# bacon205/Multimodal_eeg_fmri

Hardware: AMD Instinct MI355X
Metric: pairs_per_sec_per_node (higher is better)
Workload: dtype bf16

## Files before the change

### include/mmeeg_hip.h

```cpp
#ifndef MMEEG_HIP_H
#define MMEEG_HIP_H

#include <stdint.h>

#ifdef __cplusplus
extern "C" {
#endif

typedef struct ihipStream_t* hipStream_t;

#define MM_ABI_VERSION 5

const char* mm_last_error(void);
int mm_abi_version(void);

int mm_pack_nct_bf16(const float* x, void* y, int B, int C, int T, int Cp, hipStream_t stream);
int mm_unpack_ntc_f32(const void* g, float* dx, int B, int C, int T, int Cp, hipStream_t stream);
int mm_prep_conv_weight(const float* w, void* w_fwd, void* w_dgrad, int Cout, int Cin, int k,
                        int Cinp, int Coutp, hipStream_t stream);

int mm_conv1d_fwd(const void* x, const void* w, int B, int T, int Cin, int Cout, int taps, int pad,
                  const float* scale, const float* shift, int act, const float* residual,
                  const float* pe, int pool, float* stats, float* out_f32, void* out_bf16,
                  void* out_pre, float drop_p, uint32_t drop_seed, const uint32_t* seed_epoch,
                  const void* gradz, int gradz_act, hipStream_t stream);
int mm_conv1d_fwd_splitk_plan(int B, int T, int Cin, int Cout, int taps, int* nsplit_host, int64_t* ws_floats_host,
                              hipStream_t stream);
int mm_conv1d_fwd_splitk(const void* x, const void* w, int B, int T, int Cin, int Cout, int taps, int pad,
                  const float* scale, const float* shift, int act, const float* residual,
                  const float* pe, int pool, float* stats, float* out_f32, void* out_bf16,
                  void* out_pre, float drop_p, uint32_t drop_seed, const uint32_t* seed_epoch,
                  const void* gradz, int gradz_act, float* ws, int nsplit, hipStream_t stream);
int mm_conv1d_wgrad(const void* dy, const void* x, float* dw, float* dbias, int B, int T, int Cin,
                    int Cout, int taps, int pad, int Cin_real, int64_t sn, int64_t sc, int64_t stap,
                    int nrep, int64_t rep_stride, int slot_mode, hipStream_t stream);
int mm_conv1d_wgrad_slots(int B, int T, int Cin, int Cout, int taps, int* slots_host, hipStream_t stream);
int mm_conv1d_wgrad_many(const void* desc_host, int n, hipStream_t stream);
int mm_conv1d_wgrad_many_slots(int B, int T, int Cin, int Cout, int* slots_host, hipStream_t stream);
int mm_wgrad_scatter(const float* ws, float* dw, int Cout, int Cin, int taps, int Cinp, int nrep,
                     hipStream_t stream);
int mm_add_pe(const float* x, const float* pe, float* out_f32, void* out_bf16, int B, int L, int D,
              float drop_p, uint32_t seed, const uint32_t* seed_epoch, hipStream_t stream);

int mm_debug_stamp(void* buf, int idx, hipStream_t stream);
int mm_prep_many(const void* desc_host, int ndesc, hipStream_t stream);
int mm_prep_many_zero(const void* desc_host, int ndesc, float* zero, int64_t nzero, hipStream_t stream);
int mm_scatter_many(const void* desc_host, int ndesc, hipStream_t stream);
int mm_reduce_many(const void* desc_host, int ndesc, hipStream_t stream);
int mm_flush_many(const void* scatter_desc_host, int nscatter, const void* reduce_desc_host, int nreduce,
                  hipStream_t stream);
int mm_acc_reduce(const float* acc, float* dst, int K, int64_t rep_stride, hipStream_t stream);
int mm_reduce_replicas(const float* src, float* dst, int K, int nrep, int64_t rep_stride, hipStream_t stream);

int mm_bn_finalize(const float* stats, const float* gamma, const float* beta, float* run_mean,
                   float* run_var, const float* conv_bias, float* out4, int N, float count,
                   float momentum, float eps, int mode, void* batches_tracked, hipStream_t stream);
typedef struct {
    const float* stats;
    const float* gamma; const float* beta;
    float* run_mean; float* run_var;
    float* out4;
    void* batches_tracked;
    float count, momentum, eps;
    int reserved;
} mm_bn_fin_t;
int mm_bn_act_fwd_fin(const float* y, const void* bn_fin_host, const float* pe, void* out_bf16, float* out_f32,
                      int R, int S, int N, int act, int pool, int drop_first, float drop_p, uint32_t seed,
                      float drop2_p, uint32_t seed2, const uint32_t* seed_epoch, hipStream_t stream);
int mm_bn_act_fwd_ln_fin(const float* y, const void* bn_fin_host, const float* pe, float* out_f32, int R, int S,
                         int act, float drop_p, uint32_t seed, float drop2_p, uint32_t seed2,
                         const uint32_t* seed_epoch, const float* ln_gamma, const float* ln_beta, float ln_eps,
                         void* ln_out_bf16, float* ln_stat, hipStream_t stream);
int mm_pool3d_bn_act_fwd_fin(const void* y, const void* bn_fin_host, void* out_bf16, void* ysel, void* arg, int B,
                             int D, int H, int W, int N, int act, float drop_p, uint32_t seed,
                             const uint32_t* seed_epoch, hipStream_t stream);
int mm_conv3d_l1_fwd_fin(const float* x, const void* wimg, const float* bias, const void* bn_fin_host, void* out,
                         int B, int D, int H, int W, float drop_p, uint32_t seed, const uint32_t* seed_epoch,
                         hipStream_t stream);
int mm_bn_act_fwd(const float* y, const float* scale, const float* shift, const float* pe,
                  void* out_bf16, float* out_f32, int R, int S, int N, int act, int pool,
                  int drop_first, float drop_p, uint32_t seed, float drop2_p, uint32_t seed2,
                  const uint32_t* seed_epoch, hipStream_t stream);
int mm_bn_act_fwd_ln(const float* y, const float* scale, const float* shift, const float* pe, float* out_f32,
                     int R, int S, int act, float drop_p, uint32_t seed, float drop2_p, uint32_t seed2,
                     const uint32_t* seed_epoch, const float* ln_gamma, const float* ln_beta, float ln_eps,
                     void* ln_out_bf16, float* ln_stat, hipStream_t stream);
int mm_bn_act_bwd_reduce(const float* y, const float* out4, const void* dout_bf16,
                         const float* dout_f32, float* sums_out, int R, int S, int N, int act,
                         int pool, int drop_first, float drop_p, uint32_t seed, float drop2_p,
                         uint32_t seed2, const uint32_t* seed_epoch, hipStream_t stream);
int mm_bn_act_bwd_apply(const float* y, const float* out4, const void* dout_bf16,
                        const float* dout_f32, const float* sums, void* dy, float* dy_f32, int R,
                        int S, int N, int act, int pool, int drop_first, float drop_p, uint32_t seed,
                        float drop2_p, uint32_t seed2, const uint32_t* seed_epoch, int train, int sums_nrep, hipStream_t stream);

int mm_layernorm_fwd(const float* x, const float* gamma, const float* beta, void* out_bf16,
                     float* out_f32, float* stat, int M, int D, float eps, hipStream_t stream);
int mm_layernorm_bwd(const void* dy_bf16, const float* dy_f32, const float* x, const float* stat,
                     const float* gamma, const float* dres, float* dx, void* dx_bf16, float* dgb_repl,
                     int M, int D, float drop_p, uint32_t seed, const uint32_t* seed_epoch,
                     hipStream_t stream);
int mm_linear_dgrad_ln_bwd(const void* dy, const void* w, int M, int K, const float* x, const float* stat,
                           const float* gamma, const float* dres, float* dx, void* dx_bf16, float* dgb_repl,
                           float drop_p, uint32_t seed, const uint32_t* seed_epoch, hipStream_t stream);

int mm_conv1d_dgrad_bn_reduce(const void* dy, const void* w_dgrad, int B, int T, int Cin, int Cout, int taps, int pad,
                              void* dx_bf16, const float* y_below, const float* out4_below, float* sums_below, int act,
                              int pool, int drop_first, float drop_p, uint32_t seed, const uint32_t* seed_epoch,
                              hipStream_t stream);

int mm_linear_fwd_ln_gemm2(const void* x, const void* w, int M, int K, const float* bias, const float* residual,
                           float* out_f32, float drop_p, uint32_t seed, const uint32_t* seed_epoch,
                           const float* ln_gamma, const float* ln_beta, float ln_eps, void* ln_out_bf16, float* ln_stat,
                           const void* w2, const float* bias2, int n2, void* out2_bf16, hipStream_t stream);
int mm_linear_fwd_ln_gemm2_act(const void* x, const void* w, int M, int K, const float* bias, const float* residual,
                               float* out_f32, float drop_p, uint32_t seed, const uint32_t* seed_epoch,
                               const float* ln_gamma, const float* ln_beta, float ln_eps, void* ln_out_bf16,
                               float* ln_stat, const void* w2, const float* bias2, int n2, void* out2_bf16,
                               void* pre2_bf16, int act2, float drop2_p, uint32_t seed2, hipStream_t stream);
int mm_linear_dgrad_ln_bwd_gemm2(const void* dy, const void* w, int M, int K, const float* x, const float* stat,
                                 const float* gamma, const float* dres, float* dx, void* dx_bf16, float* dgb_repl,
                                 float drop_p, uint32_t seed, const uint32_t* seed_epoch, const void* w2, void* do_bf16,
                                 int dres_rows_per_sample, hipStream_t stream);
int mm_linear_dgrad_ln_bwd_bn_reduce(const void* dy, const void* w, int M, int K, const float* x, const float* stat,
                                     const float* gamma, const float* dres, float* dx, float* dgb_repl,
                                     const uint32_t* seed_epoch, const float* y_below, const float* out4_below,
                                     float* sums_below, int act, float bn_drop_p, uint32_t bn_seed, float bn_drop2_p,
                                     uint32_t bn_seed2, hipStream_t stream);

int mm_bn_act_bwd_reduce_bcast(const float* y, const float* out4, const float* dout_rows, float scale, float* sums_out,
                               int R, int S, int N, int act, float drop_p, uint32_t seed, const uint32_t* seed_epoch,
                               hipStream_t stream);
int mm_bn_act_bwd_apply_bcast(const float* y, const float* out4, const float* dout_rows, float scale, const float* sums,
                              void* dy, int R, int S, int N, int act, float drop_p, uint32_t seed,
                              const uint32_t* seed_epoch, int train, int sums_nrep, hipStream_t stream);

int mm_pooled_head_bwd_rows(const float* dout, const void* z_pre_bf16, const float* W, void* dz_bf16, float* rows_out,
                            void* dx_bf16, int B, int L, int D, int N, int act, float drop_p, uint32_t seed,
                            float emit_drop_p, uint32_t emit_seed, const uint32_t* seed_epoch, hipStream_t stream);

int mm_attn_fwd(const void* qkv, void* out, float* lse, int B, int L, int H, int head_dim,
                float scale, float drop_p, uint32_t seed, const uint32_t* seed_epoch,
                const float* attn_mask, int attn_mask_per_head, hipStream_t stream);
int mm_attn_bwd(const void* qkv, const void* out, const void* dout, const float* lse, void* dqkv,
                float* delta_ws, int B, int L, int H, int head_dim, float scale, float drop_p,
                uint32_t seed, const uint32_t* seed_epoch, const float* attn_mask, int attn_mask_per_head,
                hipStream_t stream);
int mm_attn_fwd_hd(const void* qkv, void* out, float* lse, int B, int L, int H, int head_dim,
                   float scale, float drop_p, uint32_t seed, const uint32_t* seed_epoch,
                   const float* attn_mask, int attn_mask_per_head, hipStream_t stream);
int mm_attn_bwd_hd(const void* qkv, const void* out, const void* dout, const float* lse, void* dqkv,
                   float* delta_ws, int B, int L, int H, int head_dim, float scale, float drop_p,
                   uint32_t seed, const uint32_t* seed_epoch, const float* attn_mask, int attn_mask_per_head,
                   hipStream_t stream);

int mm_colsum(const void* a_bf16, const float* a_f32, float* out, int M, int N, hipStream_t stream);
int mm_meanpool_fwd(const float* x, float* out_f32, void* out_bf16, int B, int L, int D, hipStream_t stream);
int mm_meanpool_bwd(const float* g, float* dx, int B, int L, int D, hipStream_t stream);
int mm_stage_inputs(const float* eeg, void* eeg_packed_bf16, float* eeg_copy, int B, int C, int T, int Cp,
                    float* fmri_dst, const float* fmri_src, int64_t fmri_n, hipStream_t stream);
int mm_eeg_augment_plan(const float* x, uint32_t* plan, int64_t plan_words, int B, int C, int T, float p_noise, float p_drop,
                        int n_drop, uint32_t s_noise, uint32_t s_drop, uint32_t s_keys, hipStream_t stream);
int mm_stage_inputs_aug(const float* eeg, uint32_t* plan, int64_t plan_words, void* eeg_packed_bf16, float* eeg_out_f32,
                        int B, int C, int T, int Cp, float noise_factor, uint32_t s_gauss_a, uint32_t s_gauss_b,
                        float* fmri_dst, const float* fmri_src, int64_t fmri_n, hipStream_t stream);
int mm_act_bwd(const float* g_f32, const void* g_bf16, const void* z, void* out, int64_t n, int act,
               float drop_p, uint32_t seed, const uint32_t* seed_epoch, hipStream_t stream);

int mm_pack_volume_bf16(const float* x, void* y, int64_t nvox, int Cp, hipStream_t stream);
int mm_conv3d_fwd(const void* x, const void* w, int B, int D, int H, int W, int Cin, int Cout,
                  const float* shift, float* stats, float* out_f32, void* out_bf16, hipStream_t stream);
int mm_conv3d_wgrad(const void* dy, const void* x, float* dw, float* dbias, int B, int D, int H, int W,
                    int Cin, int Cout, int Cin_real, int64_t sn, int64_t sc, int64_t stap, int nrep,
                    int64_t rep_stride, int slot_mode, hipStream_t stream);
int mm_conv3d_wgrad_slots(int B, int D, int H, int W, int Cin, int Cout, int* slots_host, hipStream_t stream);
int mm_pool3d_bn_act_fwd(const void* y, const float* out4, void* out_bf16, void* ysel, void* arg, int B, int D,
                         int H, int W, int N, int act, float drop_p, uint32_t seed, const uint32_t* seed_epoch,
                         hipStream_t stream);
int mm_pool3d_bn_act_bwd_reduce(const void* ysel, const float* out4, const void* dout_bf16, float* sums_out,
                                int B, int D, int H, int W, int N, int act, float drop_p, uint32_t seed,
                                const uint32_t* seed_epoch, hipStream_t stream);
int mm_pool3d_bn_act_bwd_apply(const void* y, const void* arg, const float* out4, const void* dout_bf16,
                               const float* sums, void* dy, int B, int D, int H, int W, int N, int act,
                               float drop_p, uint32_t seed, const uint32_t* seed_epoch, int train, int sums_nrep,
                               hipStream_t stream);

int mm_conv3d_l1(int mode, const float* x, const void* wimg, const float* bias, const float* out4,
                 const void* dout, const float* sums, float* stats, void* out, float* dw_tapmajor,
                 float* dbias, int B, int D, int H, int W, int train, float drop_p, uint32_t seed,
                 const uint32_t* seed_epoch, hipStream_t stream);
int mm_conv3d_l1_fwd_winners(const float* x, const void* wimg, const float* bias, const float* out4, void* out,
                             void* arg, int B, int D, int H, int W, int train, float drop_p, uint32_t seed,
                             const uint32_t* seed_epoch, hipStream_t stream);
int mm_conv3d_l1_gram(const float* x, const void* wimg, const float* bias, float* gram, float* stats, int B, int D,
                      int H, int W, hipStream_t stream);
int mm_conv3d_l1_bwd(const float* x, const void* wimg, const float* bias, const float* out4, const void* dout,
                     float* sums_out, float* a1, const float* gram, float* dw, float* dbias, int B, int D,
                     int H, int W, int train, float drop_p, uint32_t seed, const uint32_t* seed_epoch,
                     hipStream_t stream);

int mm_small_linear_fwd(const float* x, const float* W, const float* bias, const float* scale,
                        const float* shift, float* y, float* pre, int B, int K, int N, int act,
                        float drop_p, uint32_t seed, const uint32_t* seed_epoch, hipStream_t stream);
int mm_small_linear_bwd(const float* dy, const float* x, const float* W, float* dx, float* dW, float* db,
                        int B, int K, int N, hipStream_t stream);
int mm_act_f32(const float* z, float* y, int64_t n, int act, float drop_p, uint32_t seed, const uint32_t* seed_epoch, hipStream_t stream);
int mm_act_bwd_f32(const float* g, const float* z, float* out, int64_t n, int act, float drop_p,
                   uint32_t seed, const uint32_t* seed_epoch, hipStream_t stream);
int mm_colstats(const float* x, float* stats, int B, int N, hipStream_t stream);
int mm_proj_heads_fwd(const float* x_e, const float* W_e, const float* b_e, const float* g_e, const float* be_e,
                      int K_e, const float* x_f, const float* W_f, const float* b_f, const float* g_f,
                      const float* be_f, int K_f, float* z1, float* hn, float* stat, float* z, float* nrm, int B,
                      int N, float eps, float drop_p, uint32_t seed_e, uint32_t seed_f,
                      const uint32_t* seed_epoch, hipStream_t stream);
int mm_proj_heads_bwd(const float* dz, const float* z, const float* nrm, const float* hn, const float* z1,
                      const float* stat, const float* x_e, const float* W_e, const float* g_e, int K_e,
                      const float* x_f, const float* W_f, const float* g_f, int K_f, float* dx_e, float* dW_e,
                      float* db_e, float* dg_e, float* dbe_e, float* dx_f, float* dW_f, float* db_f, float* dg_f,
                      float* dbe_f, int B, int N, float drop_p, uint32_t seed_e, uint32_t seed_f,
                      const uint32_t* seed_epoch, hipStream_t stream);
int mm_clip_loss_own_rows(const float* z_all, const float* logit_scale, float* scal4, float* dz_local, float* ws,
                          int B, int Bg, int N, int row0, hipStream_t stream);
int mm_clip_loss_ws_floats(int B, int Bg, int* floats_host, hipStream_t stream);
int mm_clip_loss_own_rows_grouped(const float* z_all, const int* gid_all, const float* logit_scale, float* scal4,
                                  float* dz_local, float* ws, int B, int Bg, int N, int row0, hipStream_t stream);
int mm_clip_loss_grouped_ws_floats(int B, int Bg, int* floats_host, hipStream_t stream);

#define MM_RETRIEVAL_KMAX 16
#define MM_RETRIEVAL_NMAX (1 << 20)
int mm_retrieval(const float* Q, const float* G, const int* pos, int* ranks, int* topk_idx, float* topk_score,
                 float* ws, int Nq, int Ng, int D, int k, hipStream_t stream);
int mm_retrieval_ws_floats(int Nq, int Ng, int D, int k, int* floats_host, hipStream_t stream);
int mm_retrieval_grouped(const float* Q, const float* G, const int* qgid, const int* ggid, int* ranks, float* ws,
                         int Nq, int Ng, int D, hipStream_t stream);
int mm_retrieval_grouped_ws_floats(int Nq, int Ng, int D, int* floats_host, hipStream_t stream);

typedef struct {
    float* w[3]; float* b[3]; float* gamma[3]; float* beta[3]; float* run_mean[3]; float* run_var[3];
    void* batches_tracked[3];
    float* W; float* B; float* Gamma; float* Beta; float* Run_mean; float* Run_var;
    int cin; int k[3]; int cinp; int reserved;
} mm_power_merge_t;
int mm_power_merge(const void* desc_host, int mode, hipStream_t stream);

int mm_softmax2_concat(const float* a, const float* c, const float* pa, const float* pc, float* out, int B,
                       int Ha, int Hc, hipStream_t stream);
int mm_learned_fusion(const float* f0, const float* f1, const float* f2, const float* dyn,
                      const float* logits, const float* temperature, float* fused, float* weights, int B,
                      int H, int M, hipStream_t stream);
int mm_attn_1xk(const float* p0, const float* p1, const float* p2, const float* p3, int K, const float* dctx,
                float* ctx, float* attw, float* dp0, float* dp1, float* dp2, float* dp3, int B, int E,
                int nhead, float drop_p, uint32_t seed, const uint32_t* seed_epoch, int backward,
                hipStream_t stream);
int mm_add_f32(const float* a, const float* b, float* out, int64_t n, hipStream_t stream);
int mm_attn_1x2(const float* proj_e, const float* proj_f, float* ctx, float* attw, int B, int E, int nhead,
                hipStream_t stream);
int mm_attn_1x2_train(const float* proj_e, const float* proj_f, const float* dctx, float* ctx, float* attw,
                      float* dproj_e, float* dproj_f, int B, int E, int nhead, float drop_p, uint32_t seed,
                      const uint32_t* seed_epoch, int backward, hipStream_t stream);
int mm_learned_fusion_bwd(const float* f0, const float* f1, const float* f2, const float* dyn,
                          const float* logits, const float* temperature, const float* dfused, float* df0,
                          float* df1, float* df2, float* ddyn, float* dlogits, float* dtemp, int B, int H,
                          int M, hipStream_t stream);
int mm_softmax2_concat_bwd(const float* dout, const float* a, const float* c, const float* pa,
                           const float* pc, float* da, float* dc, float* dpa, float* dpc, int B, int Ha,
                           int Hc, hipStream_t stream);
int mm_weighted_ce(const float* logits, const void* target_i64, const float* class_weight, float* loss_out,
                   float* dlogits, int B, int C, hipStream_t stream);
int mm_focal_loss(const float* logits, const void* target_i64, float* loss_out, float* per_sample,
                  float* dlogits, int B, int C, float alpha, float gamma, float scale, hipStream_t stream);
int mm_gate2_mix(const float* g, const float* erp, const float* pw, const float* conn, float* comb,
                 float* gate, int B, int H, float boost, hipStream_t stream);
int mm_gate2_mix_bwd(const float* dcomb, const float* g, const float* erp, const float* pw, float* derp,
                     float* dpw, float* dconn, float* dg, int B, int H, float boost, hipStream_t stream);
int mm_smoothed_ce(const float* logits, const void* target_i64, float* loss_out, float* dlogits, int B,
                   int C, float smoothing, hipStream_t stream);
int mm_stft_power(const float* x, void* out_bf16, float* out_f32, int B, int C, int T, int nfft, int hop,
                  int ch_off, int ch_total, hipStream_t stream);
#define MM_ZSCORE_WS_DOUBLES 64
int mm_sample_zscore_bf16(const float* x, void* out_bf16, double* ws, int B, int rows, int ch_valid, int ch_total,
                          float eps, hipStream_t stream);
int mm_sample_zscore_bwd(const float* x, const void* g_bf16, float* dx, int B, int rows, int ch_valid, int ch_total,
                         float eps, hipStream_t stream);
int mm_stft_power_bwd(const float* x, const float* g_power, float* dx, int B, int C, int T, int nfft, int hop,
                      int ch_off, int ch_total, hipStream_t stream);
int mm_mul_f32(const float* a, const float* b, float* out, int64_t n, hipStream_t stream);
int mm_linear_fwd_meanpool(const void* x, const void* w, int M, int K, const float* bias, const float* residual,
                           float* out_f32, float drop_p, uint32_t seed, const uint32_t* seed_epoch, float* pool_out,
                           int rows_per_group, hipStream_t stream);
int mm_linear_fwd_ln(const void* x, const void* w, int M, int K, const float* bias, const float* residual,
                     float* out_f32, float drop_p, uint32_t seed, const uint32_t* seed_epoch, const float* ln_gamma,
                     const float* ln_beta, float ln_eps, void* ln_out_bf16, float* ln_stat, hipStream_t stream);
int mm_pooled_head_fwd(const float* pooled, const float* pooled_acc, const float* W, const float* bias, float* out, void* z_pre_bf16,
                       void* pooled_bf16, int B, int D, int N, int act, float drop_p, uint32_t seed,
                       const uint32_t* seed_epoch, hipStream_t stream);
int mm_pooled_head_bwd(const float* dout, const void* z_pre_bf16, const float* W, void* dz_bf16, float* dx,
                       void* dx_bf16, int B, int L, int D, int N, int act, float drop_p, uint32_t seed,
                       float emit_drop_p, uint32_t emit_seed, const uint32_t* seed_epoch, hipStream_t stream);
int mm_drop_path(const float* x, float* out, int64_t B, int64_t inner, float drop_p, uint32_t seed,
                 const uint32_t* seed_epoch, hipStream_t stream);
int mm_meanpool_bf16(const void* x, float* out, int R, int S, int N, hipStream_t stream);

#define MM_OPT_STATE_FLOATS 1032
int mm_sumsq(const float* g, float* state, int64_t n, hipStream_t stream);
int mm_adamw_clip(float* p, float* g, float* m, float* v, float* state, int64_t n, float beta1,
                  float beta2, float eps, float weight_decay, float max_norm, float grad_scale,
                  int zero_grad, uint32_t* seed_epoch, hipStream_t stream);

int mm_xai_interp(const float* x, const float* base, int base_rows, float* out, int n_steps, int s0, int steps,
                  int64_t rows, int64_t inner, hipStream_t stream);
int mm_xai_accum(const float* grad, float* acc, int steps, int64_t n, hipStream_t stream);
int mm_xai_finish(const float* x, const float* base, int base_rows, const float* acc, float* attr, float* chan,
                  int B, int C, int64_t T, int n_steps, int mode, hipStream_t stream);
int mm_xai_pair_score(const float* z, float* score, float* seed, int B, int N, hipStream_t stream);

int mm_gatv2_fwd(const float* xl, const float* xr, int ld, const float* att, const float* bias, const int* rowptr,
                 const int* col, float* out, float* pre, float* alpha, int B, int N, int H, int C, int E,
                 float slope, int act, float drop_p, uint32_t seed, const uint32_t* seed_epoch, hipStream_t stream);
int mm_gatv2_bwd(const float* dout, const float* pre, const float* xl, const float* xr, int ld, const float* att,
                 const float* alpha, const int* rowptr, const int* col, const int* colptr, const int* row,
                 const int* perm, float* dxl, float* dxr, float* datt, float* dbias, float* ds_ws, float* dz_ws,
                 float* part_ws, int B, int N, int H, int C, int E, float slope, int act, float drop_p,
                 uint32_t seed, const uint32_t* seed_epoch, hipStream_t stream);

int mm_gatv2_edge_fwd(const float* xl, const float* xr, int ld, const float* att, const float* bias,
                      const float* w_edge, const float* edge_attr, int ea_batched, const int* rowptr, const int* col,
                      float* out, float* pre, float* alpha, int B, int N, int H, int C, int E, int D, float slope,
                      int act, float drop_p, uint32_t seed, const uint32_t* seed_epoch, hipStream_t stream);
int mm_gatv2_edge_bwd(const float* dout, const float* pre, const float* xl, const float* xr, int ld, const float* att,
                      const float* w_edge, const float* edge_attr, int ea_batched, const float* alpha,
                      const int* rowptr, const int* col, const int* colptr, const int* row, const int* perm,
                      float* dxl, float* dxr, float* datt, float* dbias, float* dw_edge, float* dedge_attr,
                      float* ds_ws, float* dz_ws, float* part_ws, float* wpart_ws, float* epart_ws, int B, int N,
                      int H, int C, int E, int D, float slope, int act, float drop_p, uint32_t seed,
                      const uint32_t* seed_epoch, hipStream_t stream);
int mm_gatv2_edge_pack(const float* listed, const int* eid, const int* rowptr, const int* indeg, float* csr, int Bo,
                       int N, int El, int E, int D, int fill_mean, float fill_value, hipStream_t stream);
int mm_gatv2_edge_pack_bwd(const float* dcsr, const int* pos, const int* tgt, const int* rowptr, const int* indeg,
                           float* dlisted, int Bo, int N, int El, int E, int D, int fill_mean, hipStream_t stream);

#ifdef __cplusplus
}
#endif
#endif
```

### multimodal_eeg_fmri_amd/autograd.py

```python
from __future__ import annotations

import os
from typing import Dict, List, Optional

import torch

from . import _hip
from . import ops
from .ops import ACT, AREPL, REPL, WREP, _BF, _F32, _empty, _zeros


_BAG = {"cur": None}


def _reduce_into(dst, src, K, stride, offset=0, nrep=REPL):
    if dst is None:
        return
    if nrep not in (1, REPL):
        raise ValueError("_reduce_into: nrep is 1 (fp32 vector) or REPL (accumulator workspace)")
    bag = _BAG["cur"]
    ptr = src.data_ptr() + (8 if nrep == REPL else 4) * offset
    if bag is not None:
        bag.defer(ptr, dst, K, AREPL if nrep == REPL else 1, stride, keep=src)
    elif nrep == REPL:
# ... 20 lines not shown
    if window is None:
        return (ws.data_ptr(), dw.data_ptr(), cout, cin, taps, cinp, nrep, 0)
    n0, tap0, ws_taps, ws_cout = window
    return (ws.data_ptr() + 4 * n0 * ws_taps * cinp, dw.data_ptr(), cout, cin, taps | (tap0 << 8) | (ws_taps << 16), cinp, nrep, ws_cout)


def _wgrad_slots(dy, x, dw, dbr, B, T, cinp, N, k, pad, cin, parts=None):
    bag = _BAG["cur"]
    grouped = bag is not None and k == 1
    if grouped:
        slots = _hip.host_int("mm_conv1d_wgrad_many_slots", B, T, cinp, N)
    else:
        slots = _hip.host_int("mm_conv1d_wgrad_slots", B, T, cinp, N, k)
    ws = _empty((slots, N, k, cinp), _F32, dy)
    if grouped:
        bag.defer_wgrad(dy, x, ws, dbr, B, T, cinp, N, slots)
    elif bag is not None and bag.defer_conv_wgrads:
        bag.calls.append(("mm_conv1d_wgrad", (dy, x, ws, dbr, B, T, cinp, N, k, pad, cinp, k * cinp, 1, cinp,
                                              slots, N * k * cinp, 1)))
    else:
        _hip.call("mm_conv1d_wgrad", dy, x, ws, dbr, B, T, cinp, N, k, pad, cinp, k * cinp, 1, cinp,
                  slots, N * k * cinp, 1)
    if parts is None:
        _scatter_into(dw, ws, N, cin, k, cinp, slots)
    else:
        for t, n0, cn, kk in parts:
            if t is not None:
                _scatter_into(t, ws, cn, cin, kk, cinp, slots, window=(n0, (k - kk) // 2, k, N))


class deferred:

    def __init__(self, bag, device):
        self.bag, self.device = bag, device

    def __enter__(self):
        self.prev = _BAG["cur"]
        _BAG["cur"] = self.bag
        return self.bag

    def __exit__(self, *exc):
        _BAG["cur"] = self.prev
        if exc[0] is None:
            self.bag.flush(self.device)
        return False


def _ln_param_grads(bag, ln, dgb, D):
    gw, gb = bag.target(ln.weight), bag.target(ln.bias)
    if gw is not None and gb is not None and gw.data_ptr() + 4 * D == gb.data_ptr():
        _reduce_into(gw, dgb, 2 * D, 2 * D)
        return
    _reduce_into(gw, dgb, D, 2 * D, 0)
    _reduce_into(gb, dgb, D, 2 * D, D)


def _compact(rep_buf, K):
    out = _zeros((K,), rep_buf)
    _hip.call("mm_acc_reduce", rep_buf, out, K, K)
    return out


def _bn_param_grads(bag, bn, sums, N, nrep=1):
    _reduce_into(bag.target(bn.bias), sums, N, 2 * N, 0, nrep=nrep)
    _reduce_into(bag.target(bn.weight), sums, N, 2 * N, N, nrep=nrep)


class GradBag:

    def __init__(self):
        self.fresh: Dict[int, torch.Tensor] = {}
        self.pending = []
        self.scatters = []
        self.wgrads = []
        self.calls = []
        self.defer_conv_wgrads = False
        self._keep = []

    def defer(self, src_ptr: int, dst: torch.Tensor, K: int, nrep: int, stride: int, keep=None):
        self.pending.append((src_ptr, dst.data_ptr(), K, nrep, stride))
        self._keep.append((dst, keep))

    def defer_scatter(self, ws: torch.Tensor, dw: torch.Tensor, cout, cin, taps, cinp, nrep, window=None):
        self.scatters.append(scatter_desc(ws, dw, cout, cin, taps, cinp, nrep, window))
        self._keep.append((dw, ws))

    def defer_wgrad(self, dy, x, ws, dbr, B, T, cinp, N, slots):
        self.wgrads.append((dy.data_ptr(), x.data_ptr(), ws.data_ptr(), dbr.data_ptr() if dbr is not None else 0,
                            B, T, cinp, N, cinp, slots))
        self._keep.append((dy, x, ws, dbr))

    def hand_over(self) -> "GradBag":
        other = GradBag()
        other.pending, other.scatters, other.wgrads, other._keep = self.pending, self.scatters, self.wgrads, self._keep
        other.calls = self.calls
        self.pending, self.scatters, self.wgrads, self.calls, self._keep = [], [], [], [], []
        return other

    def flush(self, device):
        import ctypes
        import struct
        for name, args in self.calls:
            _hip.call(name, *args)
        self._keep.append(self.calls)
        self.calls = []
        if self.wgrads:
            raw = b"".join(struct.pack("<QQQQiiiiiiii", *d, 0, 0) for d in self.wgrads)
            host = ctypes.create_string_buffer(raw, len(raw))
            _hip.call("mm_conv1d_wgrad_many", ctypes.addressof(host), len(self.wgrads))
            self.wgrads = []
        if not self.scatters and not self.pending:
            return
        sraw = b"".join(struct.pack("<QQiiiiii", *d) for d in self.scatters)
        rraw = b"".join(struct.pack("<QQqqq", *d) for d in self.pending)
        shost = ctypes.create_string_buffer(sraw, max(len(sraw), 1))
        rhost = ctypes.create_string_buffer(rraw, max(len(rraw), 1))
        _hip.call("mm_flush_many", ctypes.addressof(shost) if self.scatters else None, len(self.scatters),
                  ctypes.addressof(rhost) if self.pending else None, len(self.pending))
        self.scatters, self.pending = [], []

    def target(self, p: torch.Tensor) -> Optional[torch.Tensor]:
        if p is None or not p.requires_grad:
            return None
        sink = getattr(p, "_mm_grad", None)
        if sink is not None:
            return sink
        t = self.fresh.get(id(p))
        if t is None:
            t = torch.zeros_like(p, dtype=_F32, memory_format=torch.contiguous_format)
            self.fresh[id(p)] = t
        return t

    def result(self, p: torch.Tensor) -> Optional[torch.Tensor]:
        return self.fresh.get(id(p))


def _mask_cast(g_f32=None, g_bf16=None, z=None, act="none", drop_p=0.0, seed=0):
    src = g_f32 if g_f32 is not None else g_bf16
    out = _empty(src.shape, _BF, src)
    _hip.call("mm_act_bwd", g_f32, g_bf16, z, out, src.numel(), ACT[act], float(drop_p), int(seed), ops.EP())
    return out


def linear_bwd(bag: GradBag, dy: torch.Tensor, x: torch.Tensor, weight, bias, *, need_dx=True,
               dx_f32=False, below=None):
    """dy (M, N) bf16, x (M, Kp) bf16 -> dx (M, Kp); accumulates dW, db."""
    M, N = dy.shape
    Kp = x.shape[1]
    K = weight.shape[1]
    dw = bag.target(weight)
    db = bag.target(bias)
    dbr = _zeros((REPL, N), dy) if db is not None else None
    if dw is not None:
        _wgrad_slots(dy, x, dw, dbr, 1, M, Kp, N, 1, 0, K)
    elif db is not None:
        _hip.call("mm_colsum", dy, None, dbr, M, N)
    if db is not None:
        _reduce_into(db, dbr, N, N)
    if not need_dx:
        return None
    _, wd, cinp, coutp = ops.weights.get(weight, True)
    if coutp != N:
        raise _hip.HipLibraryError(f"linear_bwd: dY width {N} != padded out width {coutp}")
    kw = {}
    if below is not None:
        z, act, p, seed = below
        kw = dict(gradz=z, gradz_act=act, drop_p=p, seed=seed)
    r = ops.igemm(dy.view(1, M, N), wd, 1, 0, cinp, out_f32=dx_f32, out_bf16=not dx_f32, **kw)
    return (r["f32"] if dx_f32 else r["bf16"]).view(M, cinp)


_NO_BCAST = bool(os.environ.get("MM_NO_BCAST"))
_NO_GEMM2 = bool(os.environ.get("MM_NO_GEMM2"))
_NO_BNRED = bool(os.environ.get("MM_NO_BNRED"))


def _bn_bwd_args(s: dict, y):
    B, T, N = y.shape
    d2 = s.get("drop2", (0.0, 0))
    return (B, T, N, ACT[s["act"]], s["pool"], 1 if s["drop_first"] else 0, float(s["drop_p"]), int(s["seed"]),
            float(d2[0]), int(d2[1]), ops.EP())


def conv_bn_act_bwd(bag: GradBag, s: dict, dout_bf16=None, dout_f32=None, need_dx=True, sums=None, below=None):
    conv, bn = s["conv"], s["bn"]
    y, out4, xb = s["y"], s["out4"], s["xb"]
    B, T, N = y.shape
    args = _bn_bwd_args(s, y)
    if sums is None:
        sums = _zeros((REPL, 2, N), y)
        _hip.call("mm_bn_act_bwd_reduce", y, out4, dout_bf16, dout_f32, sums, *args)
    dy = _empty((B, T, N), _BF, y)
    _hip.call("mm_bn_act_bwd_apply", y, out4, dout_bf16, dout_f32, sums, dy, None, *args,
              1 if s.get("train", True) else 0, REPL)
    _bn_param_grads(bag, bn, sums, N, nrep=REPL)
    k, pad = conv.kernel_size[0], conv.padding[0]
    cin = conv.in_channels
    parts = getattr(conv, "parts", None)
    if parts is not None:
        parts = [(bag.target(w), n0, w.shape[0], w.shape[2]) for w, n0 in parts]
        dw = None
    else:
        dw = bag.target(conv.weight)
    if dw is not None or (parts is not None and any(t is not None for t, *_ in parts)):
        cinp_x = xb.shape[2]
        db = bag.target(conv.bias)
        dbr = _zeros((REPL, N), y) if db is not None else None
        _wgrad_slots(dy, xb, dw, dbr, B, T, cinp_x, N, k, pad, cin, parts=parts)
        if db is not None:
            _reduce_into(db, dbr, N, N)
    if not need_dx:
        return None if below is None else (None, None)
    _, wd, cinp, coutp = ops.weights.get(conv.weight, True)
    assert coutp == N
    if below is not None:
        yb = below["y"]
        d2 = below.get("drop2", (0.0, 0))
        if not _NO_BNRED and (k > 1 or cinp <= 64) and yb.shape[2] == cinp and yb.shape[1] == T * below["pool"] and float(d2[0]) == 0.0:
            dx = _empty((B, T, cinp), _BF, y)
            sums_b = _zeros((REPL, 2, cinp), y)
            _hip.call("mm_conv1d_dgrad_bn_reduce", dy, wd, B, T, N, cinp, k, k - 1 - pad, dx, yb, below["out4"], sums_b,
                      ACT[below["act"]], below["pool"], 1 if below["drop_first"] else 0, float(below["drop_p"]),
                      int(below["seed"]), ops.EP())
            return dx, sums_b
        return ops.igemm(dy, wd, k, k - 1 - pad, cinp)["bf16"], None
    return ops.igemm(dy, wd, k, k - 1 - pad, cinp)["bf16"]


def _linear_ln_bwd(bag, dy, h, lin, wb, x, stat, ln, dres, dx, dx_bf16, dgb, drop_p, seed, bn_below=None, gemm2=None,
                   res_rows=0):
    weight, bias = (lin.weight, lin.bias) if lin is not None else wb
    M, D = x.shape
    if D == 128 and M % 32 == 0:
        linear_bwd(bag, dy, h, weight, bias, need_dx=False)
        _, wd, cinp, coutp = ops.weights.get(weight, True)
        if coutp != dy.shape[1] or cinp != D:
            raise _hip.HipLibraryError(f"linear_ln_bwd: dY width {dy.shape[1]} / LN width {D} != weight image {coutp} x {cinp}")
        if bn_below is not None and dx_bf16 is None and dx is not None and not _NO_BNRED:
            sb = bn_below["s"]
            yb = sb["y"]
            d2 = sb.get("drop2", (0.0, 0))
            if yb.shape[2] == 128 and sb["pool"] == 1 and yb.shape[0] * yb.shape[1] == M:
                sums_b = _zeros((REPL, 2, 128), yb)
                _hip.call("mm_linear_dgrad_ln_bwd_bn_reduce", dy, wd, M, coutp, x, stat, ln.weight, dres, dx, dgb, ops.EP(),
                          yb, sb["out4"], sums_b, ACT[sb["act"]], float(sb["drop_p"]), int(sb["seed"]), float(d2[0]), int(d2[1]))
                bn_below["sums"] = sums_b
                return
        if gemm2 is not None and dx_bf16 is not None and not _NO_GEMM2:
            w2, holder = gemm2
            do = _empty((M, 128), _BF, dy)
            _hip.call("mm_linear_dgrad_ln_bwd_gemm2", dy, wd, M, coutp, x, stat, ln.weight, dres, dx, dx_bf16, dgb,
                      drop_p, seed, ops.EP(), w2, do, int(res_rows))
            holder.append(do)
            return
        _hip.call("mm_linear_dgrad_ln_bwd", dy, wd, M, coutp, x, stat, ln.weight, dres, dx, dx_bf16, dgb,
                  drop_p, seed, ops.EP())
        return
    dh = linear_bwd(bag, dy, h, weight, bias)
    _hip.call("mm_layernorm_bwd", dh, None, x, stat, ln.weight, dres, dx, dx_bf16, dgb, M, D, drop_p, seed, ops.EP())


def transformer_block_bwd(bag: GradBag, s: dict, dx2: torch.Tensor, dy2=None, emit_for=None, bn_below=None):
    blk = s["blk"]
    p = s["p"]
    s1, s2, s3 = s["seeds"]
    B, L = s["B"], s["L"]
    at = blk.self_attn
    res_rows = 0
    if isinstance(dx2, tuple):
        rows, per = dx2
        M, D = dy2.shape
        _, _, ci, co = ops.weights.get(at.out_proj.weight, True)
        if D == 128 and M % 32 == 0 and ci == 128 and co == 128 and not _NO_GEMM2:
            dx2, res_rows = rows, per
        else:
            dx2 = rows.view(-1, 1, D).expand(-1, per, D).reshape(M, D).contiguous()
    else:
        M, D = dx2.shape
    if dy2 is None:
        dy2 = _mask_cast(g_f32=dx2, drop_p=p, seed=s3)
    dz = linear_bwd(bag, dy2, s["g"], blk.linear2.weight, blk.linear2.bias, below=(s["z"], blk._act, p, s2))
    dx1 = _empty((M, D), _F32, dx2)
    dyo = _empty((M, D), _BF, dx2)
    dgb = _zeros((REPL, 2, D), dx2)
    holder = []
    g2 = None
    if D == 128 and M % 32 == 0:
        _, wd_o, cinp_o, coutp_o = ops.weights.get(at.out_proj.weight, True)
        if cinp_o == 128 and coutp_o == 128:
            g2 = (wd_o, holder)
    _linear_ln_bwd(bag, dz, s["h2"], blk.linear1, None, s["x1"], s["st2"], blk.norm2, dx2, dx1, dyo, dgb,
                   float(p), int(s1), gemm2=g2, res_rows=res_rows)
    _ln_param_grads(bag, blk.norm2, dgb, D)
    if holder:
        do = holder[0]
        linear_bwd(bag, dyo, s["o"].view(M, D), at.out_proj.weight, at.out_proj.bias, need_dx=False)
    else:
        do = linear_bwd(bag, dyo, s["o"].view(M, D), at.out_proj.weight, at.out_proj.bias)
    dqkv = _empty((B, L, 3 * D), _BF, dx2)
    delta = _empty((B, blk.nhead, L), _F32, dx2)
    dh = D // blk.nhead
    pa, sa = s.get("attn_drop", (0.0, 0))
    entry = ops.attn_entry(D, blk.nhead, "bwd")
    _hip.call(entry, s["qkv"], s["o"], do, s["lse"], dqkv, delta, B, L, blk.nhead, dh, float(dh) ** -0.5,
              float(pa), int(sa), ops.EP(), s.get("mask"), ops.attn_mask_per_head(s.get("mask"), B, blk.nhead, L))
    dx0 = _empty((M, D), _F32, dx2)
    emit = _empty((M, D), _BF, dx2) if emit_for is not None else None
    ep, es = emit_for if emit_for is not None else (0.0, 0)
    dgb = _zeros((REPL, 2, D), dx2)
    _linear_ln_bwd(bag, dqkv.view(M, 3 * D), s["h1"], None, (at.in_proj_weight, at.in_proj_bias), s["x"], s["st1"],
                   blk.norm1, dx1, dx0, emit, dgb, float(ep), int(es), bn_below=bn_below)
    _ln_param_grads(bag, blk.norm1, dgb, D)
    return dx0, emit


def pooled_head_bwd(bag: GradBag, s: dict, dout: torch.Tensor, emit_for=None, rows_only=False):
    lin = s["lin"]
    if s.get("fused") and rows_only and emit_for is None and not _NO_BCAST:
        B, L, D = s["B"], s["L"], s["D"]
        N = lin.weight.shape[0]
        dout = dout.contiguous()
        dz = _empty((B, N), _BF, dout)
        dp = _empty((B, 1, D), _F32, dout)
        _hip.call("mm_pooled_head_bwd", dout, s["z"], lin.weight, dz, dp, None, B, 1, D, N, ACT[s["act"]],
                  float(s["drop_p"]), int(s["seed"]), 0.0, 0, ops.EP())
        linear_bwd(bag, dz, s["pooled"], lin.weight, lin.bias, need_dx=False)
        return dp.view(B, D), 1.0 / L
    if s.get("fused") and rows_only and emit_for is not None and not _NO_BCAST:
        B, L, D = s["B"], s["L"], s["D"]
        N = lin.weight.shape[0]
        dout = dout.contiguous()
        dz = _empty((B, N), _BF, dout)
        rows = _empty((B, D), _F32, dout)
        emit = _empty((B, L, D), _BF, dout)
        _hip.call("mm_pooled_head_bwd_rows", dout, s["z"], lin.weight, dz, rows, emit, B, L, D, N, ACT[s["act"]],
                  float(s["drop_p"]), int(s["seed"]), float(emit_for[0]), int(emit_for[1]), ops.EP())
        linear_bwd(bag, dz, s["pooled"], lin.weight, lin.bias, need_dx=False)
        return (rows, L), emit
    if s.get("fused"):
        B, L, D = s["B"], s["L"], s["D"]
        N = lin.weight.shape[0]
        dout = dout.contiguous()
        dz = _empty((B, N), _BF, dout)
        dx = _empty((B, L, D), _F32, dout)
        emit = _empty((B, L, D), _BF, dout) if emit_for is not None else None
        ep, es = emit_for if emit_for is not None else (0.0, 0)
        _hip.call("mm_pooled_head_bwd", dout, s["z"], lin.weight, dz, dx, emit, B, L, D, N, ACT[s["act"]],
                  float(s["drop_p"]), int(s["seed"]), float(ep), int(es), ops.EP())
        linear_bwd(bag, dz, s["pooled"], lin.weight, lin.bias, need_dx=False)
        return (dx, emit) if emit_for is not None else dx
    if emit_for is not None:
        return pooled_head_bwd(bag, s, dout), None
    dz = _mask_cast(g_f32=dout.contiguous(), z=s["z"], act=s["act"], drop_p=s["drop_p"], seed=s["seed"])
    dpool = linear_bwd(bag, dz, s["pooled"], lin.weight, lin.bias, dx_f32=True)
    B, L, D = s["B"], s["L"], s["D"]
    dx = _empty((B, L, D), _F32, dout)
    _hip.call("mm_meanpool_bwd", dpool, dx, B, L, D)
    return dx


def _module_params(m) -> List[torch.nn.Parameter]:
    return [p for p in m.parameters()]


class _ModuleFn(torch.autograd.Function):

    @staticmethod
    def _finish(ctx, bag, params, dx):
        return (None, dx) + tuple(bag.result(p) for p in params)


def erp_encoder_bwd(bag: GradBag, sv: dict, dout: torch.Tensor, need_dx: bool = False, after_blocks=None,
                    after_conv2=None, after_conv3=None):
    blocks = sv["blocks"]
    dy2 = None
    if blocks:
        d, dy2 = pooled_head_bwd(bag, sv["head"], dout, emit_for=(blocks[-1]["p"], blocks[-1]["seeds"][2]), rows_only=True)
    else:
        d = pooled_head_bwd(bag, sv["head"], dout)
    if isinstance(d, tuple):
        B, L, D = dy2.shape
    else:
        B, L, D = d.shape
        d = d.view(B * L, D)
    if dy2 is not None:
        dy2 = dy2.view(B * L, D)
    c3, c2, c1 = sv["convs"][2], sv["convs"][1], sv["convs"][0]
    bn3 = {"s": c3}
    for i in range(len(blocks) - 1, -1, -1):
        below = (blocks[i - 1]["p"], blocks[i - 1]["seeds"][2]) if i > 0 else None
        d, dy2 = transformer_block_bwd(bag, blocks[i], d, dy2=dy2, emit_for=below, bn_below=bn3 if i == 0 else None)
    if after_blocks is not None:
        after_blocks()
    g, sm = conv_bn_act_bwd(bag, c3, dout_f32=d.view(B, L, D), sums=bn3.get("sums"), below=c2)
    if after_conv3 is not None:
        after_conv3()
    g, sm = conv_bn_act_bwd(bag, c2, dout_bf16=g, sums=sm, below=c1)
    if after_conv2 is not None:
        after_conv2()
    g = conv_bn_act_bwd(bag, c1, dout_bf16=g, need_dx=need_dx, sums=sm)
    if not need_dx:
        return None
    Bx, C, T = sv["x_shape"]
    dx = _empty((Bx, C, T), _F32, dout)
    _hip.call("mm_unpack_ntc_f32", g, dx, Bx, C, T, g.shape[2])
    return dx


class ErpEncoderFn(_ModuleFn):

    @staticmethod
    def run(m, x):
        return ErpEncoderFn.apply(m, x, *_module_params(m))

    @staticmethod
    def forward(ctx, m, x, *params):
        out, saved = ops._erp_forward_impl(m, x.float(), m.training, True, save=True)
        ctx.m, ctx.saved, ctx.params = m, saved, params
        ctx.need_dx = x.requires_grad
        return out

    @staticmethod
    def backward(ctx, dout):
        bag = GradBag()
        with deferred(bag, dout.device):
            dx = erp_encoder_bwd(bag, ctx.saved, dout, ctx.need_dx)
        return _ModuleFn._finish(ctx, bag, ctx.params, dx)


def power_encoder_bwd(bag: GradBag, sv: dict, dout: torch.Tensor, need_dx: bool = False):
    d = pooled_head_bwd(bag, sv["head"], dout)
    B, L, D = d.shape
    d = d.view(B * L, D)
    blocks = sv["blocks"]
    dy2 = None
    for i in range(len(blocks) - 1, -1, -1):
        below = (blocks[i - 1]["p"], blocks[i - 1]["seeds"][2]) if i > 0 else None
        d, dy2 = transformer_block_bwd(bag, blocks[i], d, dy2=dy2, emit_for=below)
    g = conv_bn_act_bwd(bag, sv["convs"][1], dout_f32=d.view(B, L, D))
    g = conv_bn_act_bwd(bag, sv["convs"][0], dout_bf16=g, need_dx=need_dx)
    conv, bn, seqs = sv["merged"]

    def finish():
        tg = lambda ps: [bag.target(p) for p in ps]
        none3 = [None] * 3
        ops.power_merge_call(2, (tg([sq[0].weight for sq in seqs]), tg([sq[0].bias for sq in seqs]), tg([sq[1].weight for sq in seqs]),
                                 tg([sq[1].bias for sq in seqs]), none3, none3),
                             [bag.result(conv.weight), bag.result(conv.bias), bag.result(bn.weight), bag.result(bn.bias), None, None],
                             cin=conv.in_channels, ks=[sq[0].kernel_size[0] for sq in seqs])
    return g, finish


class PowerEncoderFn(_ModuleFn):

    @staticmethod
    def run(m, x, packed=False):
        return PowerEncoderFn.apply(m, x, packed, *_module_params(m))

    @staticmethod
    def forward(ctx, m, x, packed, *params):
        xb = x if packed else ops.pack_nct(x.float())
        need_dx = bool(x.requires_grad)
        out, saved = ops._power_forward_impl(m, xb, m.training, need_dx, save=True)
        ctx.saved, ctx.params = saved, params
        ctx.need_dx, ctx.x_shape, ctx.packed = need_dx, tuple(x.shape), bool(packed)
        return out

    @staticmethod
    def backward(ctx, dout):
        bag = GradBag()
        with deferred(bag, dout.device):
            g, finish = power_encoder_bwd(bag, ctx.saved, dout.contiguous(), ctx.need_dx)
        finish()
        dx = None
        if ctx.need_dx and ctx.packed:
            dx = g
        elif ctx.need_dx:
            Bx, C, T = ctx.x_shape
            dx = _empty((Bx, C, T), _F32, dout)
            _hip.call("mm_unpack_ntc_f32", g, dx, Bx, C, T, g.shape[2])
        return (None, dx, None) + tuple(bag.result(p) for p in ctx.params)


class StftFrontEndFn(torch.autograd.Function):

    @staticmethod
    def forward(ctx, x, n_ffts, hop, normalize):
        xc = x.float().contiguous()
        out, spec = ops.stft_front_end(xc, n_ffts, hop, normalize, keep_spec=True)
        ctx.save_for_backward(xc, spec if spec is not None else out)
        ctx.cfg = (tuple(n_ffts), int(hop), bool(normalize))
        return out

    @staticmethod
    def backward(ctx, g):
        xc, spec = ctx.saved_tensors
        n_ffts, hop, normalize = ctx.cfg
        B, C, T = xc.shape
        frames, cp = g.shape[1], g.shape[2]
        widths = [C * (n // 2 + 1) for n in n_ffts]
        g = g.contiguous()
        if normalize:
            gp = _empty((B, frames, cp), _F32, g)
            _hip.call("mm_sample_zscore_bwd", spec, g, gp, B, frames, sum(widths), cp, 1e-8)
        else:
            gp = g.float()
        dx = torch.zeros_like(xc)
        off = 0
        for n, wdt in zip(n_ffts, widths):
            _hip.call("mm_stft_power_bwd", xc, gp, dx, B, C, T, int(n), hop, off, cp)
            off += wdt
        return dx, None, None, None


class AddPositionalFn(torch.autograd.Function):

    @staticmethod
    def forward(ctx, x, pe, p):
        seed = ops._next_seed() if p > 0 else 0
        ctx.p, ctx.seed, ctx.dtype = p, seed, x.dtype
        return ops.add_positional_impl(x, pe, p, seed)

    @staticmethod
    def backward(ctx, dout):
        if ctx.p > 0:
            dx = ops.add_positional_impl(dout, None, ctx.p, ctx.seed, backward=True)
        else:
            dx = dout
        return dx.to(ctx.dtype), None, None


class TransformerBlockFn(_ModuleFn):
    @staticmethod
    def run(blk, x, mask=None):
        return TransformerBlockFn.apply(blk, x, mask, *_module_params(blk))

    @staticmethod
    def forward(ctx, blk, x, mask, *params):
        xf = x.float().contiguous()
        out, saved = ops.transformer_block_fwd(xf, blk, blk.training, True, save=True, mask=mask)
        ctx.blk, ctx.saved, ctx.params = blk, saved, params
        return out

    @staticmethod
    def backward(ctx, dout):
        bag = GradBag()
        B, L, D = dout.shape
        with deferred(bag, dout.device):
            dx, _ = transformer_block_bwd(bag, ctx.saved, dout.contiguous().view(B * L, D).float())
        return (None, dx.view(B, L, D), None) + tuple(bag.result(p) for p in ctx.params)


def conv3d_bn_act_bwd(bag: GradBag, s: dict, dout, need_dx=True):
    conv, bn = s["conv"], s["bn"]
    y, out4, xv = s["y"], s["out4"], s["xv"]
    B, D, H, W, N = y.shape
    train = 1 if s.get("train", True) else 0
    sums = _zeros((REPL, 2, N), y)
    dy = _empty((B, D, H, W, N), _BF, y)
    gelu = ACT["gelu"]
    if s["pool"]:
        _hip.call("mm_pool3d_bn_act_bwd_reduce", s["ysel"], out4, dout, sums, B, D, H, W, N, gelu,
                  float(s["drop_p"]), int(s["seed"]), ops.EP())
        _hip.call("mm_pool3d_bn_act_bwd_apply", y, s["arg"], out4, dout, sums, dy, B, D, H, W, N, gelu,
                  float(s["drop_p"]), int(s["seed"]), ops.EP(), train, REPL)
    elif isinstance(dout, tuple):
        rows, scale = dout
        _hip.call("mm_bn_act_bwd_reduce_bcast", y, out4, rows, float(scale), sums, B, D * H * W, N, gelu,
                  float(s["drop_p"]), int(s["seed"]), ops.EP())
        _hip.call("mm_bn_act_bwd_apply_bcast", y, out4, rows, float(scale), sums, dy, B, D * H * W, N, gelu,
                  float(s["drop_p"]), int(s["seed"]), ops.EP(), train, REPL)
    else:
        args = (B, D * H * W, N, gelu, 1, 1, float(s["drop_p"]), int(s["seed"]), 0.0, 0, ops.EP())
        _hip.call("mm_bn_act_bwd_reduce", y, out4, None, dout, sums, *args)
        _hip.call("mm_bn_act_bwd_apply", y, out4, None, dout, sums, dy, None, *args, train, REPL)
    _bn_param_grads(bag, bn, sums, N, nrep=REPL)
    cin = conv.in_channels
    dw = bag.target(conv.weight)
    if dw is not None:
        cinp_x = xv.shape[4]
        db = bag.target(conv.bias)
        dbr = _zeros((REPL, N), y) if db is not None else None
        slots = _hip.host_int("mm_conv3d_wgrad_slots", B, D, H, W, cinp_x, N)
        ws = _empty((slots, N, 27, cinp_x), _F32, y)
        end = ops.kernel_timer.bracket(f"conv3d_wgrad_c{cinp_x}")
        _hip.call("mm_conv3d_wgrad", dy, xv, ws, dbr, B, D, H, W, cinp_x, N, cinp_x,
                  27 * cinp_x, 1, cinp_x, slots, N * 27 * cinp_x, 1)
        if end is not None:
            end.record()
        _scatter_into(dw, ws, N, cin, 27, cinp_x, slots)
        if db is not None:
            _reduce_into(db, dbr, N, N)
    if not need_dx:
        return None
    _, wd, cinp, coutp = ops.weights.get(conv.weight, True)
    assert coutp == N
    dx = _empty((B, D, H, W, cinp), _BF, y)
    end = ops.kernel_timer.bracket(f"conv3d_dgrad_c{N}")
    _hip.call("mm_conv3d_fwd", dy, wd, B, D, H, W, N, cinp, None, None, None, dx)
    if end is not None:
        end.record()
    return dx


def conv3d_l1_bwd(bag: GradBag, s: dict, dout: torch.Tensor):
    conv, bn, x = s["conv"], s["bn"], s["x"]
    B, _, D, H, W = x.shape
    train = 1 if s.get("train", True) else 0
# ... 125 lines not shown
```

### multimodal_eeg_fmri_amd/csrc/attention.hip

```cpp
#include "common.h"

namespace {

constexpr int VR = 32;

__device__ __forceinline__ bf16x8 tr_frag32(const bf16* tile, int row0, int lane) {
    const int li = lane & 15, g = lane >> 4;
    const bf16* p = tile + (row0 + 8 * (g >> 1) + (li >> 2)) * VR + (g & 1) * 16 + 4 * (li & 3);
    typedef __attribute__((address_space(3))) s16x4 lds_s16x4;
    union { s16x4 s[2]; bf16x8 v; } u;
    u.s[0] = __builtin_amdgcn_ds_read_tr16_b64_v4i16((lds_s16x4*)(p));
    u.s[1] = __builtin_amdgcn_ds_read_tr16_b64_v4i16((lds_s16x4*)(p + 4 * VR));
    return u.v;
}

__device__ __forceinline__ int vperm(int key) {
    return (key & ~12) | ((key & 4) << 1) | ((key & 8) >> 1);
}

__device__ __forceinline__ uint32_t attn_block_hash(uint32_t seed, int bh, int q, int key, int L) {
    const uint32_t Lh = ((uint32_t)L + 1u) >> 1;
    uint32_t x = (((uint32_t)bh * Lh + ((uint32_t)q >> 1)) * Lh + ((uint32_t)key >> 1)) * 0x9E3779B1u + seed;
    x ^= x >> 13;
    x = __umul24(x, 0xB5297Bu);
    x ^= x >> 15;
    return x;
}
template <bool ALONG_KEYS>
__device__ __forceinline__ void attn_keep2(uint32_t seed, int bh, int mine, int other, int L, uint32_t thresh8, bool& k0, bool& k1) {
    if (ALONG_KEYS) {
        const uint32_t x = attn_block_hash(seed, bh, mine, other, L) >> (16 * (mine & 1));
        k0 = (x & 0xFFu) >= thresh8;
        k1 = ((x >> 8) & 0xFFu) >= thresh8;
    } else {
        const uint32_t x = attn_block_hash(seed, bh, other, mine, L) >> (8 * (mine & 1));
        k0 = (x & 0xFFu) >= thresh8;
        k1 = ((x >> 16) & 0xFFu) >= thresh8;
    }
}

__device__ __forceinline__ float xhalf_max(float v) {
    const auto r = __builtin_amdgcn_permlane32_swap(__float_as_uint(v), __float_as_uint(v), false, false);
    return fmaxf(__uint_as_float(r[0]), __uint_as_float(r[1]));
}
__device__ __forceinline__ float xhalf_sum(float v) {
    const auto r = __builtin_amdgcn_permlane32_swap(__float_as_uint(v), __float_as_uint(v), false, false);
    return __uint_as_float(r[0]) + __uint_as_float(r[1]);
}

__device__ __forceinline__ float fast_exp2(float x) { return __builtin_amdgcn_exp2f(x); }

__device__ __forceinline__ void zero8(bf16x8& v) {
#pragma unroll
    for (int j = 0; j < 8; ++j) v[j] = (bf16)0.f;
}

constexpr int KCH = 128;
constexpr int QCH = 128;

template <int DHP>
struct Hd {
    static_assert(DHP == 32 || DHP == 64, "padded head width");
    static constexpr int NS = DHP / 16;
    static constexpr int NT = DHP / 32;
    static constexpr int KS = DHP + 8;
    static constexpr int NG = DHP / 8;
    static __device__ __forceinline__ int tr_off(int rows, int row, int sg) { return (sg >> 2) * rows * VR + row * VR + (sg & 3) * 8; }
};

template <int DHP, bool EXACT>
struct Dims {
    int L, H, dh_;
    Dims(int L, int H, int dh) : L(L), H(H), dh_(dh) {}
    __device__ int dh() const { return dh_; }
};
template <int DHP>
struct Dims<DHP, true> {
    int L, H;
    Dims(int L, int H, int) : L(L), H(H) {}
    __device__ constexpr int dh() const { return DHP; }
};

template <int DHP, bool EXACT, bool DROP, bool FULL, bool MASK>
__global__ __launch_bounds__(256) void attn_fwd_kernel(const bf16* __restrict__ qkv, bf16* __restrict__ out,
                                                       float* __restrict__ lse, const Dims<DHP, EXACT> dm, float scale_log2,
                                                       uint32_t dthresh, uint32_t dseed, float dinv,
                                                       const uint32_t* epoch, const float* __restrict__ amask, size_t amask_bh) {
    using T = Hd<DHP>;
    constexpr int NS = T::NS, NT = T::NT, KS = T::KS, NG = T::NG;
    const int L = dm.L, H = dm.H, dh = dm.dh();
    dseed = mm_eff_seed(dseed, epoch);
    if (MASK) amask += (size_t)(blockIdx.z * H + blockIdx.y) * amask_bh;
    __shared__ __attribute__((aligned(16))) bf16 Ks[KCH * KS];
    __shared__ __attribute__((aligned(16))) bf16 Vs[NT * KCH * VR];
    const int E = H * dh, E3 = 3 * E;
    const int b = blockIdx.z, h = blockIdx.y;
    const int tid = threadIdx.x, lane = tid & 63, wave = tid >> 6;
    const int lr = lane & 31, lh = lane >> 5;
    const int q = blockIdx.x * 128 + wave * 32 + lr;
    const bf16* base = qkv + (size_t)b * L * E3 + h * dh;

    bf16x8 qf[NS];
#pragma unroll
    for (int s = 0; s < NS; ++s) {
        zero8(qf[s]);
        if (q < L && 16 * s + 8 * lh < dh) qf[s] = *reinterpret_cast<const bf16x8*>(base + (size_t)q * E3 + 16 * s + 8 * lh);
    }
    f32x16 o[NT];
#pragma unroll
    for (int t = 0; t < NT; ++t)
#pragma unroll
        for (int r = 0; r < 16; ++r) o[t][r] = 0.f;
    float m_run = -INFINITY, l_run = 0.f;

    constexpr int NI = KCH * NG / 256;
    uint4 kreg[NI], vreg[NI];
    auto load_chunk = [&](int k0) __attribute__((always_inline)) {
        const int kn = min(KCH, L - k0);
#pragma unroll
        for (int i = 0; i < NI; ++i) {
            const int s = tid + i * 256, key = s / NG, sg = s % NG;
            kreg[i] = make_uint4(0, 0, 0, 0); vreg[i] = make_uint4(0, 0, 0, 0);
            if (key < kn && sg * 8 < dh) {
                const bf16* row = base + (size_t)(k0 + key) * E3;
                kreg[i] = *reinterpret_cast<const uint4*>(row + E + sg * 8);
                vreg[i] = *reinterpret_cast<const uint4*>(row + 2 * E + sg * 8);
            }
        }
    };
    load_chunk(0);
#pragma unroll
    for (int s = 0; s < NS; ++s) asm volatile("" : : "v"(qf[s]));
    for (int k0 = 0; k0 < L; k0 += KCH) {
        const int kn = min(KCH, L - k0);
        const int kn32 = (kn + 31) & ~31;
        __syncthreads();
#pragma unroll
        for (int i = 0; i < NI; ++i) {
            const int s = tid + i * 256, key = s / NG, sg = s % NG;
            if (key >= kn32) continue;
            *reinterpret_cast<uint4*>(Ks + key * KS + sg * 8) = kreg[i];
            *reinterpret_cast<uint4*>(Vs + T::tr_off(KCH, vperm(key), sg)) = vreg[i];
        }
        __syncthreads();
        if (k0 + KCH < L) load_chunk(k0 + KCH);
        bf16x8 kfr[NS];
#pragma unroll
        for (int s = 0; s < NS; ++s) kfr[s] = *reinterpret_cast<const bf16x8*>(Ks + lr * KS + 16 * s + 8 * lh);
        for (int kt = 0; kt < kn32; kt += 32) {
            f32x16 sacc;
#pragma unroll
            for (int r = 0; r < 16; ++r) sacc[r] = 0.f;
#pragma unroll
            for (int s = 0; s < NS; ++s) sacc = __builtin_amdgcn_mfma_f32_32x32x16_bf16(kfr[s], qf[s], sacc, 0, 0, 0);
            bf16x8 vfr[NT][2];
#pragma unroll
            for (int t = 0; t < NT; ++t)
#pragma unroll
                for (int s = 0; s < 2; ++s) vfr[t][s] = tr_frag32(Vs + t * KCH * VR, kt + 16 * s, lane);
            if (kt + 32 < kn32)
#pragma unroll
                for (int s = 0; s < NS; ++s) kfr[s] = *reinterpret_cast<const bf16x8*>(Ks + (kt + 32 + lr) * KS + 16 * s + 8 * lh);
            const float sc2 = MASK ? 1.f : scale_log2;
            float mx = -INFINITY;
#pragma unroll
            for (int r = 0; r < 16; ++r) {
                const int key = kt + (r & 3) + 8 * (r >> 2) + 4 * lh;
                float sc = sacc[r];
                if (MASK) {
                    sc *= scale_log2;
                    if (key < kn) sc += amask[(size_t)min(q, L - 1) * L + k0 + key] * 1.4426950408889634f;
                }
                sacc[r] = (FULL || key < kn) ? sc : -INFINITY;
                mx = fmaxf(mx, sacc[r]);
            }
            mx = xhalf_max(mx);
            if (__builtin_amdgcn_ballot_w64(mx * sc2 > m_run + 8.f)) {
                const float m_new = fmaxf(m_run, mx * sc2);
                const float alpha = fast_exp2(m_run - ((MASK && m_new == -INFINITY) ? 0.f : m_new));
                l_run *= alpha;
                m_run = m_new;
#pragma unroll
                for (int t = 0; t < NT; ++t)
#pragma unroll
                    for (int r = 0; r < 16; ++r) o[t][r] *= alpha;
            }
            const float m_neg = (MASK && m_run == -INFINITY) ? 0.f : -m_run;
            float ps = 0.f;
            union { bf16x8 v[2]; bf16x2 h[8]; } pu;
#pragma unroll
            for (int r = 0; r < 16; r += 2) {
                float p0 = fast_exp2(fmaf(sacc[r], sc2, m_neg)), p1 = fast_exp2(fmaf(sacc[r + 1], sc2, m_neg));
                ps += p0;
                ps += p1;
                if (DROP) {
                    bool kp0, kp1;
                    attn_keep2<true>(dseed, b * H + h, q, k0 + kt + (r & 3) + 8 * (r >> 2) + 4 * lh, L, dthresh, kp0, kp1);
                    p0 = kp0 ? p0 : 0.f; p1 = kp1 ? p1 : 0.f;
                }
                typedef __attribute__((ext_vector_type(2))) float f32x2_t;
                pu.h[r >> 1] = __builtin_convertvector((f32x2_t){p0, p1}, bf16x2);
            }
            l_run += ps;
#pragma unroll
            for (int t = 0; t < NT; ++t)
#pragma unroll
                for (int s = 0; s < 2; ++s) o[t] = __builtin_amdgcn_mfma_f32_32x32x16_bf16(vfr[t][s], pu.v[s], o[t], 0, 0, 0);
        }
    }
    const float l_tot = xhalf_sum(l_run);
    const float inv = (DROP ? dinv : 1.f) / l_tot;
    if (q < L) {
        bf16* orow = out + ((size_t)b * L + q) * E + h * dh;
#pragma unroll
        for (int t = 0; t < NT; ++t)
#pragma unroll
            for (int g = 0; g < 4; ++g) {
                const int d = 32 * t + 8 * g + 4 * lh;
                if (d >= dh) continue;
                bf16x4 v = {(bf16)(o[t][4 * g] * inv), (bf16)(o[t][4 * g + 1] * inv), (bf16)(o[t][4 * g + 2] * inv), (bf16)(o[t][4 * g + 3] * inv)};
                *reinterpret_cast<bf16x4*>(orow + d) = v;
            }
        if (lse && lh == 0) lse[((size_t)b * H + h) * L + q] = (m_run + log2f(l_tot)) * 0.6931471805599453f;
    }
}

template <int DHP, bool EXACT, bool DROP, bool FULL, bool MASK>
__global__ __launch_bounds__(256) void attn_bwd_dq_kernel(const bf16* __restrict__ qkv, const bf16* __restrict__ out,
                                                          const bf16* __restrict__ dout, const float* __restrict__ lse,
                                                          bf16* __restrict__ dqkv, float* __restrict__ delta,
                                                          const Dims<DHP, EXACT> dm, float scale, uint32_t dthresh,
                                                          uint32_t dseed, float dinv, const uint32_t* epoch,
                                                          const float* __restrict__ amask, size_t amask_bh) {
    using T = Hd<DHP>;
    constexpr int NS = T::NS, NT = T::NT, KS = T::KS, NG = T::NG;
    const int L = dm.L, H = dm.H, dh = dm.dh();
    dseed = mm_eff_seed(dseed, epoch);
    if (MASK) amask += (size_t)(blockIdx.z * H + blockIdx.y) * amask_bh;
    __shared__ __attribute__((aligned(16))) bf16 Ks[KCH * KS];
    __shared__ __attribute__((aligned(16))) bf16 Vs[KCH * KS];
    __shared__ __attribute__((aligned(16))) bf16 Kr[NT * KCH * VR];
    const int E = H * dh, E3 = 3 * E;
    const int b = blockIdx.z, h = blockIdx.y;
    const int tid = threadIdx.x, lane = tid & 63, wave = tid >> 6;
    const int lr = lane & 31, lh = lane >> 5;
    const int q = blockIdx.x * 128 + wave * 32 + lr;
    const bool qok = q < L;
    const bf16* base = qkv + (size_t)b * L * E3 + h * dh;
    const float scale_log2 = scale * 1.4426950408889634f;

    bf16x8 qf[NS], dof[NS];
    float dl = 0.f;
#pragma unroll
    for (int s = 0; s < NS; ++s) {
        zero8(qf[s]); zero8(dof[s]);
        if (qok && 16 * s + 8 * lh < dh) {
            qf[s] = *reinterpret_cast<const bf16x8*>(base + (size_t)q * E3 + 16 * s + 8 * lh);
            const size_t oi = ((size_t)b * L + q) * E + h * dh + 16 * s + 8 * lh;
            dof[s] = *reinterpret_cast<const bf16x8*>(dout + oi);
            const bf16x8 of = *reinterpret_cast<const bf16x8*>(out + oi);
#pragma unroll
            for (int j = 0; j < 8; ++j) dl += (float)dof[s][j] * (float)of[j];
        }
    }
    dl = xhalf_sum(dl);
    const float lse2 = qok ? lse[((size_t)b * H + h) * L + q] * 1.4426950408889634f : 0.f;
    if (qok && lh == 0) delta[((size_t)b * H + h) * L + q] = dl;

    f32x16 dq[NT];
#pragma unroll
    for (int t = 0; t < NT; ++t)
#pragma unroll
        for (int r = 0; r < 16; ++r) dq[t][r] = 0.f;

    constexpr int NI = KCH * NG / 256;
    uint4 kreg[NI], vreg[NI];
    auto load_chunk = [&](int k0) __attribute__((always_inline)) {
        const int kn = min(KCH, L - k0);
#pragma unroll
        for (int i = 0; i < NI; ++i) {
            const int s = tid + i * 256, key = s / NG, sg = s % NG;
            kreg[i] = make_uint4(0, 0, 0, 0); vreg[i] = make_uint4(0, 0, 0, 0);
            if (key < kn && sg * 8 < dh) {
                const bf16* row = base + (size_t)(k0 + key) * E3;
                kreg[i] = *reinterpret_cast<const uint4*>(row + E + sg * 8);
                vreg[i] = *reinterpret_cast<const uint4*>(row + 2 * E + sg * 8);
            }
        }
    };
    load_chunk(0);
#pragma unroll
    for (int s = 0; s < NS; ++s) asm volatile("" : : "v"(qf[s]), "v"(dof[s]));
    asm volatile("" : : "v"(dl), "v"(lse2));
    for (int k0 = 0; k0 < L; k0 += KCH) {
        const int kn = min(KCH, L - k0);
        const int kn32 = (kn + 31) & ~31;
        __syncthreads();
#pragma unroll
        for (int i = 0; i < NI; ++i) {
            const int s = tid + i * 256, key = s / NG, sg = s % NG;
            if (key >= kn32) continue;
            *reinterpret_cast<uint4*>(Ks + key * KS + sg * 8) = kreg[i];
            *reinterpret_cast<uint4*>(Vs + key * KS + sg * 8) = vreg[i];
            *reinterpret_cast<uint4*>(Kr + T::tr_off(KCH, vperm(key), sg)) = kreg[i];
        }
        __syncthreads();
        if (k0 + KCH < L) load_chunk(k0 + KCH);
        for (int kt = 0; kt < kn32; kt += 32) {
            f32x16 sacc, dp;
#pragma unroll
            for (int r = 0; r < 16; ++r) { sacc[r] = 0.f; dp[r] = 0.f; }
            bf16x8 kfr[NS], vfr[NS];
#pragma unroll
            for (int s = 0; s < NS; ++s) {
                kfr[s] = *reinterpret_cast<const bf16x8*>(Ks + (kt + lr) * KS + 16 * s + 8 * lh);
                vfr[s] = *reinterpret_cast<const bf16x8*>(Vs + (kt + lr) * KS + 16 * s + 8 * lh);
            }
#pragma unroll
            for (int s = 0; s < NS; ++s) {
                sacc = __builtin_amdgcn_mfma_f32_32x32x16_bf16(kfr[s], qf[s], sacc, 0, 0, 0);
                dp = __builtin_amdgcn_mfma_f32_32x32x16_bf16(vfr[s], dof[s], dp, 0, 0, 0);
            }
            bf16x8 ktfr[NT][2];
#pragma unroll
            for (int t = 0; t < NT; ++t)
#pragma unroll
                for (int s = 0; s < 2; ++s) ktfr[t][s] = tr_frag32(Kr + t * KCH * VR, kt + 16 * s, lane);
            bf16x8 dsf[2];
            bool kp[16];
            if (DROP)
#pragma unroll
                for (int r = 0; r < 16; r += 2)
                    attn_keep2<true>(dseed, b * H + h, q, k0 + kt + (r & 3) + 8 * (r >> 2) + 4 * lh, L, dthresh, kp[r], kp[r + 1]);
#pragma unroll
            for (int r = 0; r < 16; ++r) {
                const int key = kt + (r & 3) + 8 * (r >> 2) + 4 * lh;
                float sc = fmaf(sacc[r], scale_log2, -lse2);
                if (MASK && key < kn) sc += amask[(size_t)min(q, L - 1) * L + k0 + key] * 1.4426950408889634f;
                const float p = (FULL || key < kn) ? fast_exp2(sc) : 0.f;
                float dpr = dp[r];
                if (DROP) dpr = fmaf(kp[r] ? dpr : 0.f, dinv, -dl);
                else dpr -= dl;
                dsf[r >> 3][r & 7] = (bf16)(p * dpr);
            }
#pragma unroll
            for (int t = 0; t < NT; ++t)
#pragma unroll
                for (int s = 0; s < 2; ++s) dq[t] = __builtin_amdgcn_mfma_f32_32x32x16_bf16(ktfr[t][s], dsf[s], dq[t], 0, 0, 0);
        }
    }
    if (qok) {
        bf16* drow = dqkv + ((size_t)b * L + q) * E3 + h * dh;
#pragma unroll
        for (int t = 0; t < NT; ++t)
#pragma unroll
            for (int g = 0; g < 4; ++g) {
                const int d = 32 * t + 8 * g + 4 * lh;
                if (d >= dh) continue;
                bf16x4 v = {(bf16)(dq[t][4 * g] * scale), (bf16)(dq[t][4 * g + 1] * scale), (bf16)(dq[t][4 * g + 2] * scale), (bf16)(dq[t][4 * g + 3] * scale)};
                *reinterpret_cast<bf16x4*>(drow + d) = v;
            }
    }
}

template <int DHP, bool EXACT, bool DROP, bool FULL, bool MASK>
__global__ __launch_bounds__(256) void attn_bwd_dkv_kernel(const bf16* __restrict__ qkv, const bf16* __restrict__ dout,
                                                           const float* __restrict__ lse, const float* __restrict__ delta,
                                                           bf16* __restrict__ dqkv, const Dims<DHP, EXACT> dm, float scale,
                                                           uint32_t dthresh, uint32_t dseed, float dinv,
                                                           const uint32_t* epoch, const float* __restrict__ amask, size_t amask_bh) {
    using T = Hd<DHP>;
    constexpr int NS = T::NS, NT = T::NT, KS = T::KS, NG = T::NG;
    const int L = dm.L, H = dm.H, dh = dm.dh();
    dseed = mm_eff_seed(dseed, epoch);
    if (MASK) amask += (size_t)(blockIdx.z * H + blockIdx.y) * amask_bh;
    __shared__ __attribute__((aligned(16))) bf16 Qs[QCH * KS];
    __shared__ __attribute__((aligned(16))) bf16 Ds[QCH * KS];
    __shared__ __attribute__((aligned(16))) bf16 Qr[NT * QCH * VR];
    __shared__ __attribute__((aligned(16))) bf16 Dr[NT * QCH * VR];
    __shared__ float Ls[QCH], Dl[QCH];
    const int E = H * dh, E3 = 3 * E;
    const int b = blockIdx.z, h = blockIdx.y;
    const int tid = threadIdx.x, lane = tid & 63, wave = tid >> 6;
    const int lr = lane & 31, lh = lane >> 5;
    const int key = blockIdx.x * 128 + wave * 32 + lr;
    const bool kok = key < L;
    const bf16* base = qkv + (size_t)b * L * E3 + h * dh;
    const float scale_log2 = scale * 1.4426950408889634f;

    bf16x8 kf[NS], vf[NS];
#pragma unroll
    for (int s = 0; s < NS; ++s) {
        zero8(kf[s]); zero8(vf[s]);
        if (kok && 16 * s + 8 * lh < dh) {
            kf[s] = *reinterpret_cast<const bf16x8*>(base + (size_t)key * E3 + E + 16 * s + 8 * lh);
            vf[s] = *reinterpret_cast<const bf16x8*>(base + (size_t)key * E3 + 2 * E + 16 * s + 8 * lh);
        }
    }
    f32x16 dk[NT], dv[NT];
#pragma unroll
    for (int t = 0; t < NT; ++t)
#pragma unroll
        for (int r = 0; r < 16; ++r) { dk[t][r] = 0.f; dv[t][r] = 0.f; }

    constexpr int NI = QCH * NG / 256;
    static_assert(QCH <= 256, "one lse / delta value per thread");
    uint4 qreg[NI], dreg[NI];
    float lreg = INFINITY, dlreg = 0.f;
    auto load_chunk = [&](int q0) __attribute__((always_inline)) {
        const int qn = min(QCH, L - q0);
#pragma unroll
        for (int i = 0; i < NI; ++i) {
            const int s = tid + i * 256, qi = s / NG, sg = s % NG;
            qreg[i] = make_uint4(0, 0, 0, 0); dreg[i] = make_uint4(0, 0, 0, 0);
            if (qi < qn && sg * 8 < dh) {
                qreg[i] = *reinterpret_cast<const uint4*>(base + (size_t)(q0 + qi) * E3 + sg * 8);
                dreg[i] = *reinterpret_cast<const uint4*>(dout + ((size_t)b * L + q0 + qi) * E + h * dh + sg * 8);
            }
        }
        const bool ok = tid < qn;
        lreg = ok ? lse[((size_t)b * H + h) * L + q0 + tid] : INFINITY;
        dlreg = ok ? delta[((size_t)b * H + h) * L + q0 + tid] : 0.f;
    };
    load_chunk(0);
#pragma unroll
    for (int s = 0; s < NS; ++s) asm volatile("" : : "v"(kf[s]), "v"(vf[s]));
    for (int q0 = 0; q0 < L; q0 += QCH) {
        const int qn = min(QCH, L - q0);
        const int qn32 = (qn + 31) & ~31;
        __syncthreads();
#pragma unroll
        for (int i = 0; i < NI; ++i) {
            const int s = tid + i * 256, qi = s / NG, sg = s % NG;
            if (qi >= qn32) continue;
            *reinterpret_cast<uint4*>(Qs + qi * KS + sg * 8) = qreg[i];
            *reinterpret_cast<uint4*>(Ds + qi * KS + sg * 8) = dreg[i];
            *reinterpret_cast<uint4*>(Qr + T::tr_off(QCH, vperm(qi), sg)) = qreg[i];
            *reinterpret_cast<uint4*>(Dr + T::tr_off(QCH, vperm(qi), sg)) = dreg[i];
        }
        if (tid < qn32) { Ls[tid] = lreg * 1.4426950408889634f; Dl[tid] = dlreg; }
        __syncthreads();
        if (q0 + QCH < L) load_chunk(q0 + QCH);
        for (int qt = 0; qt < qn32; qt += 32) {
            f32x16 sacc, dp;
#pragma unroll
            for (int r = 0; r < 16; ++r) { sacc[r] = 0.f; dp[r] = 0.f; }
            bf16x8 qar[NS], dar[NS];
#pragma unroll
            for (int s = 0; s < NS; ++s) {
                qar[s] = *reinterpret_cast<const bf16x8*>(Qs + (qt + lr) * KS + 16 * s + 8 * lh);
                dar[s] = *reinterpret_cast<const bf16x8*>(Ds + (qt + lr) * KS + 16 * s + 8 * lh);
            }
#pragma unroll
            for (int s = 0; s < NS; ++s) {
                sacc = __builtin_amdgcn_mfma_f32_32x32x16_bf16(qar[s], kf[s], sacc, 0, 0, 0);
                dp = __builtin_amdgcn_mfma_f32_32x32x16_bf16(dar[s], vf[s], dp, 0, 0, 0);
            }
            bf16x8 dtar[NT][2], qtar[NT][2];
#pragma unroll
            for (int t = 0; t < NT; ++t)
#pragma unroll
                for (int s = 0; s < 2; ++s) {
                    dtar[t][s] = tr_frag32(Dr + t * QCH * VR, qt + 16 * s, lane);
                    qtar[t][s] = tr_frag32(Qr + t * QCH * VR, qt + 16 * s, lane);
                }
            bf16x8 pf[2], dsf[2];
            bool kp[16];
            if (DROP)
#pragma unroll
                for (int r = 0; r < 16; r += 2)
                    attn_keep2<false>(dseed, b * H + h, key, q0 + qt + (r & 3) + 8 * (r >> 2) + 4 * lh, L, dthresh, kp[r], kp[r + 1]);
#pragma unroll
            for (int r = 0; r < 16; ++r) {
                const int qi = qt + (r & 3) + 8 * (r >> 2) + 4 * lh;
                float sc = fmaf(sacc[r], scale_log2, -Ls[qi]);
                if (MASK && kok && qi < qn) sc += amask[(size_t)(q0 + qi) * L + key] * 1.4426950408889634f;
                const float p = (FULL || kok) ? fast_exp2(sc) : 0.f;
                pf[r >> 3][r & 7] = (bf16)((!DROP || kp[r]) ? p : 0.f);
                const float u = DROP ? fmaf(kp[r] ? dp[r] : 0.f, dinv, -Dl[qi]) : dp[r] - Dl[qi];
                dsf[r >> 3][r & 7] = (bf16)(p * u);
            }
#pragma unroll
            for (int t = 0; t < NT; ++t)
#pragma unroll
                for (int s = 0; s < 2; ++s) {
                    dv[t] = __builtin_amdgcn_mfma_f32_32x32x16_bf16(dtar[t][s], pf[s], dv[t], 0, 0, 0);
                    dk[t] = __builtin_amdgcn_mfma_f32_32x32x16_bf16(qtar[t][s], dsf[s], dk[t], 0, 0, 0);
                }
        }
    }
    if (kok) {
        bf16* krow = dqkv + ((size_t)b * L + key) * E3 + E + h * dh;
        bf16* vrow = krow + E;
        const float dvs = DROP ? dinv : 1.f;
#pragma unroll
        for (int t = 0; t < NT; ++t)
#pragma unroll
            for (int g = 0; g < 4; ++g) {
                const int d = 32 * t + 8 * g + 4 * lh;
                if (d >= dh) continue;
                bf16x4 a = {(bf16)(dk[t][4 * g] * scale), (bf16)(dk[t][4 * g + 1] * scale), (bf16)(dk[t][4 * g + 2] * scale), (bf16)(dk[t][4 * g + 3] * scale)};
                bf16x4 c = {(bf16)(dv[t][4 * g] * dvs), (bf16)(dv[t][4 * g + 1] * dvs), (bf16)(dv[t][4 * g + 2] * dvs), (bf16)(dv[t][4 * g + 3] * dvs)};
                *reinterpret_cast<bf16x4*>(krow + d) = a;
                *reinterpret_cast<bf16x4*>(vrow + d) = c;
            }
    }
}

uint32_t attn_thresh(float p) { return p > 0.f ? (uint32_t)((double)p * 256.0 + 0.5) : 0u; }
float attn_keep_scale(uint32_t t) { return t ? 256.f / (256.f - (float)t) : 1.f; }

bool hd_supported(int dh) { return dh >= 16 && dh <= 64 && dh % 8 == 0; }

template <int DHP, bool EXACT>
void launch_fwd(const void* qkv, void* out, float* lse, int B, int L, int H, int dh, float scale, float drop_p,
                uint32_t seed, const uint32_t* seed_epoch, const float* attn_mask, int per_head, hipStream_t st) {
    const uint32_t dth = attn_thresh(drop_p);
    const size_t mask_bh = attn_mask && per_head ? (size_t)L * L : 0;
    const bool full = L % KCH == 0;
    auto kern = dth ? (full ? attn_fwd_kernel<DHP, EXACT, true, true, false> : attn_fwd_kernel<DHP, EXACT, true, false, false>)
                    : (full ? attn_fwd_kernel<DHP, EXACT, false, true, false> : attn_fwd_kernel<DHP, EXACT, false, false, false>);
    if (attn_mask) kern = dth ? attn_fwd_kernel<DHP, EXACT, true, false, true> : attn_fwd_kernel<DHP, EXACT, false, false, true>;
    hipLaunchKernelGGL(kern, dim3(ceil_div(L, 128), H, B), dim3(256), 0, st, (const bf16*)qkv, (bf16*)out, lse,
                       Dims<DHP, EXACT>(L, H, dh), scale * 1.4426950408889634f, dth, seed, attn_keep_scale(dth), seed_epoch,
                       attn_mask, mask_bh);
}

template <int DHP, bool EXACT>
int launch_bwd(const void* qkv, const void* out, const void* dout, const float* lse, void* dqkv, float* delta_ws,
               int B, int L, int H, int dh, float scale, float drop_p, uint32_t seed, const uint32_t* seed_epoch,
               const float* attn_mask, int per_head, hipStream_t st) {
    const uint32_t dth = attn_thresh(drop_p);
    const float dinv = attn_keep_scale(dth);
    const size_t mask_bh = attn_mask && per_head ? (size_t)L * L : 0;
    const bool full = L % KCH == 0 && L % QCH == 0;
    auto kdq = dth ? (full ? attn_bwd_dq_kernel<DHP, EXACT, true, true, false> : attn_bwd_dq_kernel<DHP, EXACT, true, false, false>)
                   : (full ? attn_bwd_dq_kernel<DHP, EXACT, false, true, false> : attn_bwd_dq_kernel<DHP, EXACT, false, false, false>);
    auto kdkv = dth ? (full ? attn_bwd_dkv_kernel<DHP, EXACT, true, true, false> : attn_bwd_dkv_kernel<DHP, EXACT, true, false, false>)
                    : (full ? attn_bwd_dkv_kernel<DHP, EXACT, false, true, false> : attn_bwd_dkv_kernel<DHP, EXACT, false, false, false>);
    if (attn_mask) {
        kdq = dth ? attn_bwd_dq_kernel<DHP, EXACT, true, false, true> : attn_bwd_dq_kernel<DHP, EXACT, false, false, true>;
        kdkv = dth ? attn_bwd_dkv_kernel<DHP, EXACT, true, false, true> : attn_bwd_dkv_kernel<DHP, EXACT, false, false, true>;
    }
    const dim3 grid(ceil_div(L, 128), H, B);
    const Dims<DHP, EXACT> dm(L, H, dh);
    hipLaunchKernelGGL(kdq, grid, dim3(256), 0, st, (const bf16*)qkv, (const bf16*)out, (const bf16*)dout, lse,
                       (bf16*)dqkv, delta_ws, dm, scale, dth, seed, dinv, seed_epoch, attn_mask, mask_bh);
    int rc = mm_check_launch(EXACT ? "attn_bwd_dq" : "attn_bwd_hd_dq");
    if (rc) return rc;
    hipLaunchKernelGGL(kdkv, grid, dim3(256), 0, st, (const bf16*)qkv, (const bf16*)dout, lse, delta_ws, (bf16*)dqkv,
                       dm, scale, dth, seed, dinv, seed_epoch, attn_mask, mask_bh);
    return mm_check_launch(EXACT ? "attn_bwd_dkv" : "attn_bwd_hd_dkv");
}

}

extern "C" {

int mm_attn_fwd(const void* qkv, void* out, float* lse, int B, int L, int H, int head_dim, float scale,
                float drop_p, uint32_t seed, const uint32_t* seed_epoch, const float* attn_mask, int attn_mask_per_head,
                hipStream_t st) {
    MM_REQUIRE(drop_p >= 0.f && drop_p < 1.f, "attn_fwd: drop_p");
    MM_REQUIRE(qkv && out && B > 0 && L > 0 && H > 0, "attn_fwd: null/invalid");
    MM_REQUIRE(head_dim == 32, "attn_fwd: head_dim=%d (kernel is specialised for 32)", head_dim);
    launch_fwd<32, true>(qkv, out, lse, B, L, H, head_dim, scale, drop_p, seed, seed_epoch, attn_mask, attn_mask_per_head, st);
    return mm_check_launch("attn_fwd");
}

int mm_attn_bwd(const void* qkv, const void* out, const void* dout, const float* lse, void* dqkv, float* delta_ws,
                int B, int L, int H, int head_dim, float scale, float drop_p, uint32_t seed,
                const uint32_t* seed_epoch, const float* attn_mask, int attn_mask_per_head, hipStream_t st) {
    MM_REQUIRE(qkv && out && dout && lse && dqkv && delta_ws && B > 0 && L > 0 && H > 0, "attn_bwd: null/invalid");
    MM_REQUIRE(head_dim == 32, "attn_bwd: head_dim=%d (kernel is specialised for 32)", head_dim);
    return launch_bwd<32, true>(qkv, out, dout, lse, dqkv, delta_ws, B, L, H, head_dim, scale, drop_p, seed, seed_epoch,
                                attn_mask, attn_mask_per_head, st);
}

int mm_attn_fwd_hd(const void* qkv, void* out, float* lse, int B, int L, int H, int head_dim, float scale,
                   float drop_p, uint32_t seed, const uint32_t* seed_epoch, const float* attn_mask, int attn_mask_per_head,
                   hipStream_t st) {
    MM_REQUIRE(hd_supported(head_dim), "attn_fwd_hd: head_dim=%d (supported: multiples of 8 in [16, 64])", head_dim);
    MM_REQUIRE(drop_p >= 0.f && drop_p < 1.f, "attn_fwd_hd: drop_p");
    MM_REQUIRE(qkv && out && B > 0 && L > 0 && H > 0, "attn_fwd_hd: null/invalid");
    auto launch = head_dim <= 32 ? launch_fwd<32, false> : launch_fwd<64, false>;
    launch(qkv, out, lse, B, L, H, head_dim, scale, drop_p, seed, seed_epoch, attn_mask, attn_mask_per_head, st);
    return mm_check_launch("attn_fwd_hd");
}

int mm_attn_bwd_hd(const void* qkv, const void* out, const void* dout, const float* lse, void* dqkv, float* delta_ws,
                   int B, int L, int H, int head_dim, float scale, float drop_p, uint32_t seed,
                   const uint32_t* seed_epoch, const float* attn_mask, int attn_mask_per_head, hipStream_t st) {
    MM_REQUIRE(hd_supported(head_dim), "attn_bwd_hd: head_dim=%d (supported: multiples of 8 in [16, 64])", head_dim);
    MM_REQUIRE(drop_p >= 0.f && drop_p < 1.f, "attn_bwd_hd: drop_p");
    MM_REQUIRE(qkv && out && dout && lse && dqkv && delta_ws && B > 0 && L > 0 && H > 0, "attn_bwd_hd: null/invalid");
    auto launch = head_dim <= 32 ? launch_bwd<32, false> : launch_bwd<64, false>;
    return launch(qkv, out, dout, lse, dqkv, delta_ws, B, L, H, head_dim, scale, drop_p, seed, seed_epoch, attn_mask,
                  attn_mask_per_head, st);
}

}
```

### multimodal_eeg_fmri_amd/csrc/common.h

```cpp
#pragma once
#include <hip/hip_runtime.h>
#include <stdint.h>

typedef __bf16 bf16;
typedef __attribute__((ext_vector_type(8))) __bf16 bf16x8;
typedef __attribute__((ext_vector_type(4))) __bf16 bf16x4;
typedef __attribute__((ext_vector_type(2))) __bf16 bf16x2;
typedef __attribute__((ext_vector_type(16))) float f32x16;
typedef __attribute__((ext_vector_type(4))) float f32x4;
typedef __attribute__((ext_vector_type(4))) short s16x4;

#define MM_OK 0
#define MM_ERR_ARG (-1)
#define MM_ERR_LAUNCH (-2)
#define MM_ERR_UNSUPPORTED (-3)

#define MM_ACT_NONE 0
#define MM_ACT_GELU 1
#define MM_ACT_RELU 2
#define MM_ACT_TANH 3
#define MM_ACT_SIGMOID 4

int mm_fail(int code, const char* fmt, ...);
int mm_check_launch(const char* what);

#define MM_REQUIRE(cond, ...)                                   \
    do {                                                        \
        if (!(cond)) return mm_fail(MM_ERR_ARG, __VA_ARGS__);   \
    } while (0)

__device__ __forceinline__ void gelu_parts(float x, float& cdf, float& pdf_unnorm) {
    const float u = fabsf(x) * 0.70710678118654752f;
    const float t = __builtin_amdgcn_rcpf(1.0f + 0.3275911f * u);
    const float e = __expf(-u * u);
    const float poly = t * (0.254829592f + t * (-0.284496736f + t * (1.421413741f + t * (-1.453152027f + t * 1.061405429f))));
    const float erfa = 1.0f - poly * e;
    cdf = 0.5f * (1.0f + copysignf(erfa, x));
    pdf_unnorm = e;
}
__device__ __forceinline__ float gelu_erf(float x) {
    float cdf, e;
    gelu_parts(x, cdf, e);
    return x * cdf;
}
__device__ __forceinline__ float gelu_erf_grad(float x) {
    float cdf, e;
    gelu_parts(x, cdf, e);
    return cdf + x * 0.3989422804014327f * e;
}
__device__ __forceinline__ float apply_act(float v, int act) {
    switch (act) {
        case MM_ACT_GELU: return gelu_erf(v);
        case MM_ACT_RELU: return v > 0.f ? v : 0.f;
        case MM_ACT_TANH: return tanhf(v);
        case MM_ACT_SIGMOID: return 1.0f / (1.0f + __expf(-v));
        default: return v;
    }
}
__device__ __forceinline__ float act_grad(float z, int act) {
    switch (act) {
        case MM_ACT_GELU: return gelu_erf_grad(z);
        case MM_ACT_RELU: return z > 0.f ? 1.f : 0.f;
        case MM_ACT_TANH: { float t = tanhf(z); return 1.f - t * t; }
        case MM_ACT_SIGMOID: { float s = 1.0f / (1.0f + __expf(-z)); return s * (1.f - s); }
        default: return 1.f;
    }
}

template <int CTRL> __device__ __forceinline__ float dpp_f32(float v) {
    return __int_as_float(__builtin_amdgcn_update_dpp(0, __float_as_int(v), CTRL, 0xF, 0xF, true));
}
constexpr int DPP_XOR1 = 0xB1, DPP_XOR2 = 0x4E, DPP_HALF_MIRROR = 0x141, DPP_MIRROR = 0x140;
__device__ __forceinline__ float row16_sum(float v) {
    v += dpp_f32<DPP_XOR1>(v);
    v += dpp_f32<DPP_XOR2>(v);
    v += dpp_f32<DPP_HALF_MIRROR>(v);
    v += dpp_f32<DPP_MIRROR>(v);
    return v;
}
__device__ __forceinline__ float row16_max(float v) {
    v = fmaxf(v, dpp_f32<DPP_XOR1>(v));
    v = fmaxf(v, dpp_f32<DPP_XOR2>(v));
    v = fmaxf(v, dpp_f32<DPP_HALF_MIRROR>(v));
    v = fmaxf(v, dpp_f32<DPP_MIRROR>(v));
    return v;
}
__device__ __forceinline__ float half32_sum(float v) {
    v = row16_sum(v);
    const auto r = __builtin_amdgcn_permlane16_swap(__float_as_uint(v), __float_as_uint(v), false, false);
    return __uint_as_float(r[0]) + __uint_as_float(r[1]);
}
__device__ __forceinline__ float half32_max(float v) {
    v = row16_max(v);
    const auto r = __builtin_amdgcn_permlane16_swap(__float_as_uint(v), __float_as_uint(v), false, false);
    return fmaxf(__uint_as_float(r[0]), __uint_as_float(r[1]));
}
__device__ __forceinline__ float wave_sum(float v) {
    v = half32_sum(v);
    const auto r = __builtin_amdgcn_permlane32_swap(__float_as_uint(v), __float_as_uint(v), false, false);
    return __uint_as_float(r[0]) + __uint_as_float(r[1]);
}
__device__ __forceinline__ float wave_max(float v) {
    v = half32_max(v);
    const auto r = __builtin_amdgcn_permlane32_swap(__float_as_uint(v), __float_as_uint(v), false, false);
    return fmaxf(__uint_as_float(r[0]), __uint_as_float(r[1]));
}

__device__ __forceinline__ uint32_t mm_hash(uint32_t seed, uint32_t idx) {
    uint32_t x = idx * 0x9E3779B1u + seed;
    x ^= x >> 15;
    x *= 0x2C1B3C6Du;
    x ^= x >> 13;
    return x;
}
__device__ __forceinline__ float dropout_scale(uint32_t seed, uint32_t idx, uint32_t thresh, float inv_keep) {
    return mm_hash(seed, idx) >= thresh ? inv_keep : 0.f;
}

__device__ __forceinline__ uint32_t mm_eff_seed(uint32_t base, const uint32_t* epoch) {
    return epoch ? base ^ (epoch[0] * 0x85EBCA6Bu + 0xC2B2AE35u) : base;
}

struct DropH { uint32_t thresh; float inv_keep; };
inline DropH mm_drop(float p) {
    return p > 0.f ? DropH{(uint32_t)((double)p * 4294967296.0), 1.f / (1.f - p)} : DropH{0u, 1.f};
}

template <int ACT, int POOL, class Args>
__device__ __forceinline__ void bn_dz_pair(const Args& a, float y0, float y1, float sc, float sh, float g,
                                           uint32_t i0, uint32_t i1, uint32_t io, float& dz0, float& dz1) {
    const int act = ACT >= 0 ? ACT : a.act;
    const int pool = POOL > 0 ? POOL : a.pool;
    const float z0 = y0 * sc + sh;
    if (pool == 1) {
        float m = a.thresh ? dropout_scale(a.seed, i0, a.thresh, a.inv_keep) : 1.f;
        dz0 = g * m * act_grad(z0, act);
        dz1 = 0.f;
        return;
    }
    const float z1 = y1 * sc + sh;
    float m0 = 1.f, m1 = 1.f;
    bool first;
    if (a.thresh && a.drop_first) {
        float a0 = apply_act(z0, act), a1 = apply_act(z1, act);
        m0 = dropout_scale(a.seed, i0, a.thresh, a.inv_keep);
        m1 = dropout_scale(a.seed, i1, a.thresh, a.inv_keep);
        a0 *= m0; a1 *= m1;
        first = a0 >= a1;
    } else {
        if (a.thresh) g *= dropout_scale(a.seed, io, a.thresh, a.inv_keep);
        first = z0 >= z1;
        if (act != MM_ACT_GELU || fmaxf(z0, z1) < 0.f) first = apply_act(z0, act) >= apply_act(z1, act);
    }
    const float d = g * (first ? m0 : m1) * act_grad(first ? z0 : z1, act);
    dz0 = first ? d : 0.f;
    dz1 = first ? 0.f : d;
}


#define MM_REPL 32
#define MM_ACC_REPL 16
#define MM_ACC_STAT 28
#define MM_ACC_GRAD 40
typedef long long mm_acc_t;
#define MM_ACC_POISON (1ll << 62)
#define MM_ACC_BAD ((mm_acc_t)0x8000000000000000ull)
#define MM_ACC_MAG_LIMIT ((1u << 25) - 16u)
#ifdef __HIPCC__
template <int K> __device__ __forceinline__ void acc_add(mm_acc_t* p, float v) {
    const float f = v * (float)(1ull << K);
    if (fabsf(f) < 36028797018963968.f)
        atomicAdd(reinterpret_cast<unsigned long long*>(p), (unsigned long long)__float2ll_rn(f));
    else
        atomicExch(reinterpret_cast<unsigned long long*>(p), (unsigned long long)MM_ACC_POISON);
}
template <int K> __device__ __forceinline__ mm_acc_t acc_encode(float v) {
    const float f = v * (float)(1ull << K);
    return fabsf(f) < 2305843009213693952.f ? __float2ll_rn(f) : MM_ACC_POISON;
}
__device__ __forceinline__ unsigned acc_mag(mm_acc_t v) {
    const int hi = (int)(v >> 32);
    return (unsigned)(hi < 0 ? ~hi : hi) >> 4;
}
__device__ __forceinline__ mm_acc_t acc_guard(mm_acc_t s, unsigned mag_sum) { return mag_sum >= MM_ACC_MAG_LIMIT ? MM_ACC_BAD : s; }
template <int K> __device__ __forceinline__ float acc_val(mm_acc_t s) {
    const bool bad = (unsigned long long)(s + (1ll << 61)) >= (1ull << 62);
    return bad ? __builtin_nanf("") : (float)s * (1.0f / (float)(1ull << K));
}
__device__ __forceinline__ mm_acc_t* acc_rep(float* ws, int r, size_t n) { return reinterpret_cast<mm_acc_t*>(ws) + (size_t)r * n; }
__device__ __forceinline__ mm_acc_t acc_sum(const float* ws, size_t n, size_t i) {
    const mm_acc_t* p = reinterpret_cast<const mm_acc_t*>(ws) + i;
    mm_acc_t v[MM_ACC_REPL];
#pragma unroll
    for (int r = 0; r < MM_ACC_REPL; ++r) v[r] = p[(size_t)r * n];
    mm_acc_t s = 0;
    unsigned g = 0;
#pragma unroll
    for (int r = 0; r < MM_ACC_REPL; ++r) { s += v[r]; g += acc_mag(v[r]); }
    return acc_guard(s, g);
}
__device__ __forceinline__ mm_acc_t acc_sum_lanes16(mm_acc_t v) {
    unsigned g = acc_mag(v);
#pragma unroll
    for (int o = 8; o > 0; o >>= 1) { v += __shfl_xor(v, o, 64); g += __shfl_xor(g, o, 64); }
    return acc_guard(v, g);
}
#endif

struct MmBnFin {
    const float* stats;
    const float* gamma; const float* beta;
    float* run_mean; float* run_var;
    float* out4;
    long long* tracked;
    float count, momentum, eps;
    int N;
};
#ifdef __HIPCC__
__device__ __forceinline__ void bn_fin_channel(const MmBnFin& f, int n, bool writer, float& sc, float& sh, float& mean, float& rstd) {
    const float s1 = acc_val<MM_ACC_STAT>(acc_sum(f.stats, 2 * (size_t)f.N, n));
    const float s2 = acc_val<MM_ACC_STAT>(acc_sum(f.stats, 2 * (size_t)f.N, (size_t)f.N + n));
    mean = s1 / f.count;
    float var = s2 / f.count - mean * mean;
    var = var < 0.f ? 0.f : var;
    rstd = rsqrtf(var + f.eps);
    sc = f.gamma[n] * rstd;
    sh = f.beta[n] + (0.f - mean) * sc;
    if (writer) {
        if (n == 0 && f.tracked) f.tracked[0] += 1;
        f.run_mean[n] = (1.f - f.momentum) * f.run_mean[n] + f.momentum * mean;
        const float unb = f.count > 1.f ? var * f.count / (f.count - 1.f) : var;
        f.run_var[n] = (1.f - f.momentum) * f.run_var[n] + f.momentum * unb;
        f.out4[n] = sc; f.out4[f.N + n] = sh; f.out4[2 * f.N + n] = mean; f.out4[3 * f.N + n] = rstd;
    }
}
#endif
struct MmBnFinHost {
    const float* stats; const float* gamma; const float* beta; float* run_mean; float* run_var; float* out4;
    void* batches_tracked; float count, momentum, eps; int reserved;
};
static inline bool bn_fin_from_host(MmBnFin& f, const void* host, int N) {
    if (!host) return false;
    const MmBnFinHost& h = *static_cast<const MmBnFinHost*>(host);
    if (!h.stats || !h.gamma || !h.beta || !h.run_mean || !h.run_var || !h.out4 || !(h.count >= 1.f)) return false;
    f.stats = h.stats; f.gamma = h.gamma; f.beta = h.beta; f.run_mean = h.run_mean; f.run_var = h.run_var; f.out4 = h.out4;
    f.tracked = (long long*)h.batches_tracked; f.count = h.count; f.momentum = h.momentum; f.eps = h.eps; f.N = N;
    return true;
}

static inline int ceil_div(int a, int b) { return (a + b - 1) / b; }
static inline int grid_for(size_t n, int cap) { size_t g = (n + 255) / 256; return (int)(g < (size_t)cap ? (g ? g : 1) : cap); }

__host__ __device__ __forceinline__ bool conv3d_stream_shape(int rows, int ch) {
    return (rows == 128 && ch == 64) || (rows == 64 && ch == 128) || (rows == 32 && ch == 64);
}
__host__ __device__ __forceinline__ int conv_image_index(int rows, int k, int ch, int n, int tap, int c) {
    if (k != 27 || !conv3d_stream_shape(rows, ch)) return (n * k + tap) * ch + c;
    const int g = tap * (ch / 32) + c / 32, grp = n / 32, local = n % 32;
    return ((((g * (rows / 32) + grp) * 2 + (local & 1)) * 64 + 16 * ((c % 32) / 8) + (local >> 1)) * 8) + c % 8;
}
```

### multimodal_eeg_fmri_amd/ops.py

```python
from __future__ import annotations

import functools
import math
import os
import weakref
from typing import Dict, List, Optional

import torch

from . import _hip

ACT = {"none": 0, "gelu": 1, "relu": 2, "tanh": 3, "sigmoid": 4}
_BF = torch.bfloat16
_F32 = torch.float32


def _need_gpu(*tensors):
    for t in tensors:
        if t is not None and not t.is_cuda:
            raise _hip.HipLibraryError(
                "multimodal_eeg_fmri_amd runs on the MI355X HIP path only: got a CPU tensor "
                "(no CPU / eager-PyTorch fallback is provided)")
    _hip.load()

# ... 135 lines not shown
        self._rec = None

    def invalidate(self):
        self._gen += 1

    def start_recording(self):
        self._rec = []

    def stop_recording(self):
        rec, self._rec = self._rec or [], None
        seen, out = {}, []
        for owner, shape, dg in rec:
            k = (id(owner), shape)
            if k in seen:
                out[seen[k]][2] = out[seen[k]][2] or dg
            else:
                seen[k] = len(out)
                out.append([owner, shape, dg])
        return [tuple(e) for e in out]

    @staticmethod
    def _as3d(w: torch.Tensor) -> torch.Tensor:
        wd3 = w.detach()
        if wd3.dim() == 2:
            wd3 = wd3.unsqueeze(-1)
        if wd3.dim() == 5:
            wd3 = wd3.reshape(wd3.shape[0], wd3.shape[1], -1)
        return wd3.contiguous()

    def prepare_all(self, recorded, zero=None):
        import ctypes
        import struct
        raw, keep = [], []
        for owner, shape, need_dgrad in recorded:
            w = owner if shape is None else owner.view(shape)
            ver = (owner.data_ptr(), owner._version, self._gen, tuple(w.shape))
            hit = self._store.get(id(owner))
            if hit is not None and hit[5]() is owner and hit[0] == ver and (hit[2] is not None or not need_dgrad):
                continue
            wd3 = self._as3d(w)
            cout, cin, k3 = wd3.shape
            cinp, coutp = cpad(cin), cpad(cout)
            wf = _empty((cout, k3, cinp), _BF, w)
            wd = _empty((cinp, k3, coutp), _BF, w) if need_dgrad else None
            raw.append(struct.pack("<QQQiiiiii", wd3.data_ptr(), wf.data_ptr(), wd.data_ptr() if wd is not None else 0,
                                   cout, cin, k3, cinp, coutp if need_dgrad else 0, 0))
            keep.append(wd3)
            self._store[id(owner)] = (ver, wf, wd, cinp, coutp, weakref.ref(owner))
        if raw:
            buf = b"".join(raw)
            host = ctypes.create_string_buffer(buf, len(buf))
            if zero is not None:
                _hip.call("mm_prep_many_zero", ctypes.addressof(host), len(raw), zero[0], int(zero[1]))
            else:
                _hip.call("mm_prep_many", ctypes.addressof(host), len(raw))
        elif zero is not None:
            zero[0][:int(zero[1])].zero_()

    def seed(self, w: torch.Tensor, wf: torch.Tensor, wd, cinp: int, coutp: int):
        self._store[id(w)] = ((w.data_ptr(), w._version, self._gen, tuple(w.shape)), wf, wd, cinp, coutp, weakref.ref(w))

    def get(self, w: torch.Tensor, need_dgrad: bool, key=None):
        owner = w if key is None else key
        if self._rec is not None and not getattr(owner, "_mm_transient", False):
            self._rec.append((owner, None if key is None else tuple(w.shape), bool(need_dgrad)))
        k = id(owner)
        ver = (owner.data_ptr(), owner._version, self._gen, tuple(w.shape))
        hit = self._store.get(k)
        if (hit is not None and hit[5]() is owner and hit[0] == ver
                and (hit[2] is not None or not need_dgrad)):
            return hit[1], hit[2], hit[3], hit[4]
        wd3 = self._as3d(w)
        cout, cin, k3 = wd3.shape
        cinp, coutp = cpad(cin), cpad(cout)
        wf = _empty((cout, k3, cinp), _BF, w)
        wd = _empty((cinp, k3, coutp), _BF, w) if need_dgrad else None
        _hip.call("mm_prep_conv_weight", wd3, wf, wd, cout, cin, k3, cinp, coutp if need_dgrad else 0)
        if len(self._store) > 4096:
            self._store = {i: e for i, e in self._store.items() if e[5]() is not None}
        self._store[k] = (ver, wf, wd, cinp, coutp, weakref.ref(owner))
        return wf, wd, cinp, coutp


weights = _WeightCache()


def weights_changed():
    weights.invalidate()


def pack_nct(x: torch.Tensor) -> torch.Tensor:
    B, C, T = x.shape
    cp = cpad(C)
    y = _empty((B, T, cp), _BF, x)
    _hip.call("mm_pack_nct_bf16", x.contiguous(), y, B, C, T, cp)
    return y


AUG_PURPOSES = ("noise_decision", "drop_decision", "channel_keys", "gauss_a", "gauss_b")
_M64 = (1 << 64) - 1


def augment_streams(seed: int, step: int, rank: int = 0) -> tuple:
    out = []
    for purpose in range(len(AUG_PURPOSES)):
        z = (int(seed) * 0x9E3779B97F4A7C15 + int(step) * 0xBF58476D1CE4E5B9 + int(rank) * 0x94D049BB133111EB
             + (purpose + 1) * 0xD6E8FEB86659FD93) & _M64
        z ^= z >> 30
        z = z * 0xBF58476D1CE4E5B9 & _M64
        z ^= z >> 27
        z = z * 0x94D049BB133111EB & _M64
        z ^= z >> 31
        out.append((z ^ (z >> 32)) & 0xFFFFFFFF)
    return tuple(out)


def eeg_augment_check(B: int, C: int, T: int, n_drop: int, who: str = "eeg_augment"):
    if min(B, C, T) < 1 or C * T < 2:
        raise ValueError(f"{who}: a sample needs C * T >= 2 values for its standard deviation (got C = {C}, T = {T})")
    if B * C * ((T + 1) // 2) >= 1 << 32:
        raise ValueError(f"{who}: B * C * ceil(T / 2) must stay below 2^32 (the random stream's index)")
    if not 1 <= n_drop <= C:
        raise ValueError(f"{who}: n_drop must lie in [1, {C}] (got {n_drop})")


def eeg_augment_plan_layout(B: int, C: int, T: int):
    stride = (4 + (C + 31) // 32 + 1) & ~1
    chunk = 4096
    while (C * T + chunk - 1) // chunk > 64:
        chunk *= 2
    nchunk = (C * T + chunk - 1) // chunk
    return B * stride + 4 * B * nchunk, stride, nchunk


def eeg_augment_into(x: torch.Tensor, xb: Optional[torch.Tensor], out: Optional[torch.Tensor], *, p_noise: float, p_drop: float,
                     noise_factor: float, n_drop: int, seed: int, step: int, rank: int = 0,
                     fmri_dst: Optional[torch.Tensor] = None, fmri_src: Optional[torch.Tensor] = None,
                     plan: Optional[torch.Tensor] = None) -> torch.Tensor:
    _need_gpu(x)
    B, C, T = x.shape
    eeg_augment_check(B, C, T, n_drop)
    words, _, _ = eeg_augment_plan_layout(B, C, T)
    if plan is None:
        plan = torch.empty(words, dtype=torch.int32, device=x.device)
    s = augment_streams(seed, step, rank)
    _hip.call("mm_eeg_augment_plan", x, plan, words, B, C, T, p_noise, p_drop, n_drop, s[0], s[1], s[2])
    _hip.call("mm_stage_inputs_aug", x, plan, words, xb, out, B, C, T, cpad(C), noise_factor, s[3], s[4],
              fmri_dst, fmri_src, 0 if fmri_src is None else fmri_src.numel())
    return plan


def eeg_augment_read_plan(plan: torch.Tensor, B: int, C: int, T: int):
    _, stride, _ = eeg_augment_plan_layout(B, C, T)
    hdr = plan[:B * stride].view(B, stride)
    nw = (C + 31) // 32
    bits = (hdr[:, 4:4 + nw].unsqueeze(-1) >> torch.arange(32, device=plan.device, dtype=torch.int32)) & 1
    return hdr[:, 2] != 0, bits.reshape(B, nw * 32)[:, :C] != 0, hdr[:, 1].contiguous().view(_F32)


def eeg_augment(x: torch.Tensor, *, p_noise: float, p_drop: float, noise_factor: float, n_drop: int, seed: int, step: int,
                rank: int = 0, packed: bool = False, return_plan: bool = False):
    _need_gpu(x)
    x = x.contiguous().float()
    B, C, T = x.shape
    out = _empty((B, C, T), _F32, x)
    xb = _empty((B, T, cpad(C)), _BF, x) if packed else None
    plan = eeg_augment_into(x, xb, out, p_noise=p_noise, p_drop=p_drop, noise_factor=noise_factor, n_drop=n_drop, seed=seed,
                            step=step, rank=rank)
    res = (out, xb) if packed else out
    return (res, eeg_augment_read_plan(plan, B, C, T)) if return_plan else res


def igemm(x: torch.Tensor, wf: torch.Tensor, taps: int, pad: int, cout: int, *,
          scale=None, shift=None, act="none", residual=None, pe=None, pool=1, stats=None,
          out_f32=False, out_bf16=True, out_pre=False, drop_p=0.0, seed=0, gradz=None, gradz_act="none"):
    B, T, cin = x.shape
    res = {}
    of = _empty((B, T // pool, cout), _F32, x) if out_f32 else None
    ob = _empty((B, T // pool, cout), _BF, x) if out_bf16 else None
    op = _empty((B, T, cout), _BF, x) if out_pre else None
    args = (x, wf, B, T, cin, cout, taps, pad, scale, shift, ACT[act], residual, pe,
            pool, stats, of, ob, op, float(drop_p), int(seed), EP(), gradz, ACT[gradz_act])
    nsplit, ws_floats = _splitk_plan(B, T, cin, cout, taps)
    if nsplit > 1:
        _hip.call("mm_conv1d_fwd_splitk", *args, _empty((ws_floats,), _F32, x), nsplit)
    else:
        _hip.call("mm_conv1d_fwd", *args)
    res["f32"], res["bf16"], res["pre"] = of, ob, op
    return res


_SPLITK_PLANS: Dict[tuple, tuple] = {}


def _splitk_plan(B: int, T: int, cin: int, cout: int, taps: int):
    if taps == 1:
        return 1, 0
    key = (B, T, cin, cout, taps)
    plan = _SPLITK_PLANS.get(key)
    if plan is None:
        import ctypes
        n, ws = ctypes.c_int(0), ctypes.c_int64(0)
        _hip.call("mm_conv1d_fwd_splitk_plan", B, T, cin, cout, taps, ctypes.addressof(n), ctypes.addressof(ws))
        plan = _SPLITK_PLANS[key] = (n.value, ws.value)
    return plan


def clip_loss_ws_floats(B: int, Bg: int, grouped: bool = False) -> int:
    return _hip.host_int("mm_clip_loss_grouped_ws_floats" if grouped else "mm_clip_loss_ws_floats", B, Bg)


def clip_loss_grouped_ws_floats(B: int, Bg: int) -> int:
    return clip_loss_ws_floats(B, Bg, grouped=True)


def clip_loss_own_rows(z_all, gid_all, logit_scale1, scal, dz, B: int, row0: int):
    Bg, N2 = z_all.shape
    ws = _empty((clip_loss_ws_floats(B, Bg, gid_all is not None),), _F32, z_all)
    if gid_all is None:
        _hip.call("mm_clip_loss_own_rows", z_all, logit_scale1, scal, dz, ws, B, Bg, N2 // 2, row0)
    else:
        _hip.call("mm_clip_loss_own_rows_grouped", z_all, gid_all, logit_scale1, scal, dz, ws, B, Bg, N2 // 2, row0)


def group_ids(groups, n: int, device=None, who: str = "groups") -> Optional[torch.Tensor]:
    if groups is None:
        return None
    if not isinstance(groups, torch.Tensor):
        raise ValueError(f"{who}: group ids must be a torch.Tensor (got {type(groups).__name__})")
    if groups.dim() != 1 or groups.shape[0] != n:
        raise ValueError(f"{who}: group ids must have shape ({n},) (got {tuple(groups.shape)})")
    if groups.dtype.is_floating_point or groups.dtype.is_complex or groups.dtype == torch.bool:
        raise ValueError(f"{who}: group ids must be an integer tensor (got {groups.dtype})")
    if groups.is_cuda:
        if groups.dtype != torch.int32:
            raise ValueError(f"{who}: group ids on the device must be int32 (got {groups.dtype}); host tensors of any integer "
                             "dtype are converted")
        if device is not None and groups.device != torch.device(device):
            raise ValueError(f"{who}: group ids are on {groups.device}, the batch on {device}")
        return groups.contiguous()
    if n and groups.dtype != torch.int32:
        g64 = groups.long()
        if bool((g64 < -2 ** 31).any()) or bool((g64 >= 2 ** 31).any()):
            raise ValueError(f"{who}: group ids must fit in int32")
    g32 = groups.to(torch.int32).contiguous()
    return g32 if device is None else g32.to(device)


def linear_rows(x2d: torch.Tensor, weight: torch.Tensor, bias, *, act="none", residual=None,
                out_f32=False, out_bf16=True, out_pre=False, drop_p=0.0, seed=0, need_dgrad=False):
    M, K = x2d.shape
    wf, _, cinp, _ = weights.get(weight, need_dgrad)
    if cinp != K:
        raise _hip.HipLibraryError(f"linear: activation width {K} != padded weight width {cinp}")
    r = igemm(x2d.view(1, M, K), wf, 1, 0, weight.shape[0], shift=bias, act=act,
              residual=residual, out_f32=out_f32, out_bf16=out_bf16, out_pre=out_pre,
              drop_p=drop_p, seed=seed)
    return {k: (v.view(-1, v.shape[-1]) if v is not None else None) for k, v in r.items()}


def bn_fold_eval(bn, conv_bias) -> torch.Tensor:
    n = bn.num_features
    out4 = _empty((4, n), _F32, bn.weight)
    _hip.call("mm_bn_finalize", None, bn.weight, bn.bias, bn.running_mean, bn.running_var,
              conv_bias, out4, n, 1.0, 0.0, float(bn.eps), 1, None)
    return out4


def bn_finalize_train(bn, stats, count) -> torch.Tensor:
    n = bn.num_features
    out4 = _empty((4, n), _F32, bn.weight)
    mom = 0.1 if bn.momentum is None else float(bn.momentum)
    _hip.call("mm_bn_finalize", stats, bn.weight, bn.bias, bn.running_mean, bn.running_var,
              None, out4, n, float(count), mom, float(bn.eps), 0, bn.num_batches_tracked)
    return out4


def bn_fin_desc(bn, stats, count):
    import ctypes
    import struct
    n = bn.num_features
    out4 = _empty((4, n), _F32, bn.weight)
    mom = 0.1 if bn.momentum is None else float(bn.momentum)
    nb = bn.num_batches_tracked
    raw = struct.pack("<QQQQQQQfffi", stats.data_ptr(), bn.weight.data_ptr(), bn.bias.data_ptr(), bn.running_mean.data_ptr(),
                      bn.running_var.data_ptr(), out4.data_ptr(), nb.data_ptr() if nb is not None else 0,
                      float(count), mom, float(bn.eps), 0)
    buf = ctypes.create_string_buffer(raw, len(raw))
    return buf, out4


def layernorm(x2d: torch.Tensor, ln, want_stat: bool):
    M, D = x2d.shape
    out = _empty((M, D), _BF, x2d)
    stat = _empty((M, 2), _F32, x2d) if want_stat else None
    _hip.call("mm_layernorm_fwd", x2d, ln.weight, ln.bias, out, None, stat, M, D, float(ln.eps))
    return out, stat


def attn_effective_dropout(p: float) -> float:
    return round(256.0 * float(p)) / 256.0


def attention(qkv: torch.Tensor, nhead: int, want_lse: bool, drop_p: float = 0.0, seed: int = 0, mask=None):
    if 0.0 < float(drop_p) < 1.0 / 512.0:
        import warnings
        warnings.warn(f"attention dropout p = {drop_p} is below the kernels' resolution (1/256): no attention-probability dropout "
                      "is applied (nn.MultiheadAttention(dropout=p) would drop with probability p)")
    B, L, E3 = qkv.shape
    E = E3 // 3
    entry = attn_entry(E, nhead, "fwd")
    dh = E // nhead
    out = _empty((B, L, E), _BF, qkv)
    lse = _empty((B, nhead, L), _F32, qkv) if want_lse else None
    _hip.call(entry, qkv, out, lse, B, L, nhead, dh, 1.0 / math.sqrt(dh), float(drop_p), int(seed), EP(), mask,
              attn_mask_per_head(mask, B, nhead, L))
    return out, lse


ATTN_HEAD_DIMS = tuple(range(16, 65, 8))


def attn_entry(d_model: int, nhead: int, which: str) -> str:
    dh = d_model // nhead if nhead > 0 else 0
    if nhead <= 0 or d_model % nhead or dh not in ATTN_HEAD_DIMS:
        raise ValueError(f"self-attention: (d_model, nhead) = ({d_model}, {nhead}) gives a head dim the kernels do not run; "
                         f"supported head dims: {', '.join(map(str, ATTN_HEAD_DIMS))}")
    return f"mm_attn_{which}" if dh == 32 else f"mm_attn_{which}_hd"


def attn_mask_per_head(mask, B: int, nhead: int, L: int) -> int:
    if mask is None or mask.dim() == 2:
        return 0
    if tuple(mask.shape) != (B * nhead, L, L):
        raise ValueError(f"attn_mask: the 3-D form must be (batch * heads, L, L) = ({B * nhead}, {L}, {L}), got {tuple(mask.shape)}")
    return 1


def additive_attn_mask(mask, L: int, like: torch.Tensor):
    if mask is None:
        return None
    if mask.dim() not in (2, 3) or tuple(mask.shape[-2:]) != (L, L):
        raise ValueError(f"attn_mask: expected (L, L) or (batch * heads, L, L) with L = {L}, got {tuple(mask.shape)}")
    if mask.dtype == torch.bool:
        m = torch.zeros(tuple(mask.shape), dtype=_F32, device=like.device)
        m.masked_fill_(mask.to(like.device), float("-inf"))
        return m
    return mask.to(device=like.device, dtype=_F32).contiguous()


def conv_bn_act(xb: torch.Tensor, conv, bn, *, act="gelu", pool=1, training=False, drop_p=0.0,
                drop_first=True, pe=None, pe_drop_p=0.0, want_f32=False, want_bf16=True, need_dgrad=False,
                save=None, next_norm=None):
    save = training if save is None else save
    k = conv.kernel_size[0]
    pad = conv.padding[0]
    cout = conv.out_channels
    wf, _, cinp, _ = weights.get(conv.weight, need_dgrad)
    assert xb.shape[2] == cinp, (xb.shape, cinp)
    B, T, _ = xb.shape
    if not save:
        out4 = bn_fold_eval(bn, conv.bias)
        r = igemm(xb, wf, k, pad, cout, scale=out4[0], shift=out4[1], act=act, pe=pe, pool=pool,
                  out_f32=want_f32, out_bf16=want_bf16)
        return r, None
    stats = _zeros((REPL, 2, cout), xb) if training else None
    y = igemm(xb, wf, k, pad, cout, shift=conv.bias, stats=stats, out_f32=True, out_bf16=False)["f32"]
    fold = training and act == "gelu" and cout <= 256 and isinstance(bn.running_mean, torch.Tensor)
    fin = None
    if fold:
        fin, out4 = bn_fin_desc(bn, stats, B * T)
    else:
        out4 = bn_finalize_train(bn, stats, B * T) if training else bn_fold_eval(bn, None)
    if not training:
        drop_p = pe_drop_p = 0.0
    seed = _next_seed() if drop_p > 0 else 0
    seed2 = _next_seed() if pe_drop_p > 0 else 0
    of = _empty((B, T // pool, cout), _F32, xb) if want_f32 else None
    ob = _empty((B, T // pool, cout), _BF, xb) if want_bf16 else None
    prenorm = None
    if next_norm is not None and cout == 128 and pool == 1 and want_f32 and not want_bf16 and drop_first \
            and tuple(next_norm.normalized_shape) == (128,):
        hn = _empty((B * T, cout), _BF, xb)
        stn = _empty((B * T, 2), _F32, xb)
        if fold:
            import ctypes
            _hip.call("mm_bn_act_fwd_ln_fin", y, ctypes.addressof(fin), pe, of, B, T, ACT[act], float(drop_p), seed,
                      float(pe_drop_p), seed2, EP(), next_norm.weight, next_norm.bias, float(next_norm.eps), hn, stn)
        else:
            _hip.call("mm_bn_act_fwd_ln", y, out4[0], out4[1], pe, of, B, T, ACT[act], float(drop_p), seed,
                      float(pe_drop_p), seed2, EP(), next_norm.weight, next_norm.bias, float(next_norm.eps), hn, stn)
        prenorm = (hn, stn)
    elif fold:
        import ctypes
        _hip.call("mm_bn_act_fwd_fin", y, ctypes.addressof(fin), pe, ob, of, B, T, cout, ACT[act], pool,
                  1 if drop_first else 0, float(drop_p), seed, float(pe_drop_p), seed2, EP())
    else:
        _hip.call("mm_bn_act_fwd", y, out4[0], out4[1], pe, ob, of, B, T, cout, ACT[act], pool,
                  1 if drop_first else 0, float(drop_p), seed, float(pe_drop_p), seed2, EP())
    saved = dict(xb=xb, y=y, out4=out4, act=act, pool=pool, drop_p=drop_p, seed=seed,
                 drop2=(float(pe_drop_p), seed2), drop_first=drop_first, conv=conv, bn=bn, train=training)
    return {"f32": of, "bf16": ob, "pre": None, "prenorm": prenorm}, saved


def transformer_block_fwd(x: torch.Tensor, blk, training: bool, need_dgrad: bool = False,
                          save: Optional[bool] = None, pool_out: Optional[torch.Tensor] = None,
                          prenorm=None, next_norm=None, mask=None, next_blk=None):
    B, L, D = x.shape
    M = B * L
    save = training if save is None else save
    p = blk.dropout.p if training else 0.0
    x2 = x.view(M, D)
    fuse_ln = D == 128 and M % 32 == 0
    h1, st1 = prenorm[:2] if prenorm is not None else layernorm(x2, blk.norm1, save)
    if prenorm is not None and len(prenorm) > 2:
        qkv = prenorm[2]
    else:
        qkv = linear_rows(h1, blk.self_attn.in_proj_weight, blk.self_attn.in_proj_bias,
                          need_dgrad=need_dgrad)["bf16"]
    pa = float(blk.self_attn.dropout) if training else 0.0
    sa = _next_seed() if pa > 0 else 0
    o, lse = attention(qkv.view(B, L, 3 * D), blk.nhead, save, pa, sa, mask)
    s1 = _next_seed() if p > 0 else 0
    f1 = None
    s2 = None
    if fuse_ln:
        wf, _, cinp, _ = weights.get(blk.self_attn.out_proj.weight, need_dgrad)
        x1 = _empty((M, D), _F32, x)
        h2 = _empty((M, D), _BF, x)
        st2 = _empty((M, 2), _F32, x) if save else None
        w1, _, c1, _ = weights.get(blk.linear1.weight, need_dgrad)
        n1 = blk.linear1.weight.shape[0]
        if c1 == 128 and n1 % 128 == 0 and M * n1 < (1 << 32) and not _NO_FFN1_FUSE:
            s2 = _next_seed() if p > 0 else 0
            g1 = _empty((M, n1), _BF, x)
            z1 = _empty((M, n1), _BF, x) if save else None
            _hip.call("mm_linear_fwd_ln_gemm2_act", o.view(M, D), wf, M, cinp, blk.self_attn.out_proj.bias, x2, x1, float(p),
                      int(s1), EP(), blk.norm2.weight, blk.norm2.bias, float(blk.norm2.eps), h2, st2, w1, blk.linear1.bias,
                      n1, g1, z1, ACT[blk._act], float(p), int(s2))
            f1 = {"bf16": g1, "pre": z1, "f32": None}
        else:
            _hip.call("mm_linear_fwd_ln", o.view(M, D), wf, M, cinp, blk.self_attn.out_proj.bias, x2, x1, float(p), int(s1),
                      EP(), blk.norm2.weight, blk.norm2.bias, float(blk.norm2.eps), h2, st2)
    else:
        x1 = linear_rows(o.view(M, D), blk.self_attn.out_proj.weight, blk.self_attn.out_proj.bias,
                         residual=x2, out_f32=True, out_bf16=False, drop_p=p, seed=s1,
                         need_dgrad=need_dgrad)["f32"]
        h2, st2 = layernorm(x1, blk.norm2, save)
    if f1 is None:
        s2 = _next_seed() if p > 0 else 0
        f1 = linear_rows(h2, blk.linear1.weight, blk.linear1.bias, act=blk._act, out_pre=save,
                         drop_p=p, seed=s2, need_dgrad=need_dgrad)
    s3 = _next_seed() if p > 0 else 0
    nxt = None
    if pool_out is not None:
        wf, _, cinp, _ = weights.get(blk.linear2.weight, need_dgrad)
        x2o = _empty((M, D), _F32, x)
        _hip.call("mm_linear_fwd_meanpool", f1["bf16"], wf, M, cinp, blk.linear2.bias, x1, x2o, float(p), int(s3),
                  EP(), pool_out, L)
    elif next_norm is not None and fuse_ln:
        wf, _, cinp, _ = weights.get(blk.linear2.weight, need_dgrad)
        x2o = _empty((M, D), _F32, x)
        hn = _empty((M, D), _BF, x)
        stn = _empty((M, 2), _F32, x) if save else None
        wq = None
        if next_blk is not None and not _NO_QKV_FUSE:
            wq, _, cq, _ = weights.get(next_blk.self_attn.in_proj_weight, need_dgrad)
            if cq != 128 or next_blk.self_attn.in_proj_weight.shape[0] % 128:
                wq = None
        if wq is not None:
            nq = next_blk.self_attn.in_proj_weight.shape[0]
            qn = _empty((M, nq), _BF, x)
            _hip.call("mm_linear_fwd_ln_gemm2", f1["bf16"], wf, M, cinp, blk.linear2.bias, x1, x2o, float(p), int(s3), EP(),
                      next_norm.weight, next_norm.bias, float(next_norm.eps), hn, stn, wq, next_blk.self_attn.in_proj_bias,
                      nq, qn)
            nxt = (hn, stn, qn)
        else:
            _hip.call("mm_linear_fwd_ln", f1["bf16"], wf, M, cinp, blk.linear2.bias, x1, x2o, float(p), int(s3), EP(),
                      next_norm.weight, next_norm.bias, float(next_norm.eps), hn, stn)
            nxt = (hn, stn)
    else:
        x2o = linear_rows(f1["bf16"], blk.linear2.weight, blk.linear2.bias, residual=x1, out_f32=True,
                          out_bf16=False, drop_p=p, seed=s3, need_dgrad=need_dgrad)["f32"]
    saved = None
    if save:
        saved = dict(x=x2, h1=h1, st1=st1, qkv=qkv, o=o, lse=lse, x1=x1, h2=h2, st2=st2,
                     z=f1["pre"], g=f1["bf16"], p=p, seeds=(s1, s2, s3), attn_drop=(pa, sa), B=B, L=L, blk=blk,
                     mask=mask)
    if next_norm is not None:
        return x2o.view(B, L, D), saved, nxt
    return x2o.view(B, L, D), saved


def pooled_head_fwd(x: torch.Tensor, lin, *, act="gelu", training=False, drop_p=0.0,
                    need_dgrad=False, save=None, pooled_f32=None):
    B, L, D = x.shape
    pooled_acc = pooled_f32 is not None
    save = training if save is None else save
    p = drop_p if training else 0.0
    seed = _next_seed() if p > 0 else 0
    if D % 16 == 0 and D <= 1024:
        if pooled_f32 is None:
            pooled_f32 = _empty((B, D), _F32, x)
            _hip.call("mm_meanpool_fwd", x, pooled_f32, None, B, L, D)
        N = lin.weight.shape[0]
        out = _empty((B, N), _F32, x)
        z = _empty((B, N), _BF, x) if save else None
        pooled = _empty((B, D), _BF, x) if save else None
        _hip.call("mm_pooled_head_fwd", None if pooled_acc else pooled_f32, pooled_f32 if pooled_acc else None,
                  lin.weight, lin.bias, out, z, pooled, B, D, N, ACT[act], float(p), int(seed), EP())
        saved = dict(pooled=pooled, z=z, seed=seed, drop_p=p, B=B, L=L, D=D, lin=lin, act=act, fused=True) if save else None
        return out, saved
    pooled = _empty((B, D), _BF, x)
    _hip.call("mm_meanpool_fwd", x, None, pooled, B, L, D)
    r = linear_rows(pooled, lin.weight, lin.bias, act=act, out_f32=True, out_bf16=False,
                    out_pre=save, drop_p=p, seed=seed, need_dgrad=need_dgrad)
    saved = dict(pooled=pooled, z=r["pre"], seed=seed, drop_p=p, B=B, L=L, D=D, lin=lin,
                 act=act) if save else None
    return r["f32"], saved


def pe_table(pos_encoder, L: int) -> torch.Tensor:
    pe = pos_encoder.pe
    if L > pe.shape[0]:
        raise ValueError(f"sequence length {L} exceeds PositionalEncoding max_len {pe.shape[0]}")
    return pe[:L, 0, :].contiguous()


def _encoder_tail_impl(m, h, training: bool, need_dgrad: bool, save: bool, prenorm=None, stages=None):
    blocks = []
    B, L, D = h.shape
    nblk = len(m.transformer_layers)
    pooled = _zeros((B, 2 * D), h) if nblk and L % 32 == 0 and D == 128 else None
    layers = list(m.transformer_layers)
    for i, blk in enumerate(layers):
        if i < nblk - 1:
            h, s, prenorm = transformer_block_fwd(h, blk, training, need_dgrad, save=save, prenorm=prenorm,
                                                  next_norm=layers[i + 1].norm1, next_blk=layers[i + 1])
        else:
            h, s = transformer_block_fwd(h, blk, training, need_dgrad, save=save, pool_out=pooled, prenorm=prenorm)
        blocks.append(s)
        if stages is not None:
            stages[f"block{i}"] = h.clone()
    out, s = pooled_head_fwd(h, m.output_proj[2], training=training, drop_p=m.drop_p, need_dgrad=need_dgrad,
                             save=save, pooled_f32=pooled)
    return out, blocks, s, h


def _erp_forward_impl(m, x: torch.Tensor, training: bool, need_dgrad: bool, save=None, xb=None, stages=None):
    cl = m.conv_layers
    save = training if save is None else save
    p = m.drop_p if training else 0.0
    if xb is None:
        xb = pack_nct(x)
    saved = []
    saved_in = []
    r, s = conv_bn_act(xb, cl[0], cl[1], training=training, drop_p=p, need_dgrad=need_dgrad, save=save)
    saved.append(s)
    saved_in.append(r["bf16"])
    r, s = conv_bn_act(r["bf16"], cl[4], cl[5], pool=2, training=training, drop_p=p,
                       drop_first=False, need_dgrad=need_dgrad, save=save)
    saved.append(s)
    saved_in.append(r["bf16"])
    L = r["bf16"].shape[1]
    r, s = conv_bn_act(r["bf16"], cl[9], cl[10], training=training, drop_p=p,
                       pe=pe_table(m.pos_encoder, L), pe_drop_p=(m.pos_encoder.dropout.p if training else 0.0),
                       want_f32=True, want_bf16=False, need_dgrad=need_dgrad, save=save,
                       next_norm=m.transformer_layers[0].norm1 if len(m.transformer_layers) else None)
    saved.append(s)
    if stages is not None:
        stages["conv1"], stages["conv2"] = saved_in[0].clone(), saved_in[1].clone()
        stages["pos"] = r["f32"].clone()
        if not save:
            wf3 = weights.get(cl[9].weight, need_dgrad)[0]
            o4 = bn_fold_eval(cl[10], cl[9].bias)
            stages["conv3"] = igemm(saved_in[1], wf3, cl[9].kernel_size[0], cl[9].padding[0], cl[9].out_channels,
                                    scale=o4[0], shift=o4[1], act="gelu", out_f32=True, out_bf16=False)["f32"]
    out, blocks, s, h = _encoder_tail_impl(m, r["f32"], training, need_dgrad, save, prenorm=r.get("prenorm"), stages=stages)
    return out, dict(convs=saved, blocks=blocks, head=s, x_shape=tuple(x.shape), tokens=h)


def erp_encoder_forward(m, x: torch.Tensor) -> torch.Tensor:
    _need_gpu(x)
    if m.training or _wants_grad(m, x):
        from .autograd import ErpEncoderFn
        return ErpEncoderFn.run(m, x)
    with torch.no_grad():
        return _erp_forward_impl(m, x.float(), False, False)[0]


def _wants_grad(m, x) -> bool:
    return torch.is_grad_enabled() and (x.requires_grad or any(p.requires_grad for p in m.parameters()))


def add_positional(x, pe, drop_p, training):
    _need_gpu(x)
    if x.dim() != 3:
        raise ValueError("PositionalEncoding: expected a 3-D input (batch, seq, d_model) or (seq, 1, d_model)")
    L = x.size(1) if x.size(1) != 1 else x.size(0)
    if L > pe.shape[0]:
        raise ValueError(f"sequence length {L} exceeds PositionalEncoding max_len {pe.shape[0]}")
    from .autograd import AddPositionalFn
    return AddPositionalFn.apply(x, pe, float(drop_p) if training else 0.0)


def add_positional_impl(x, pe, p: float, seed: int, backward: bool = False):
    shape = x.shape
    if x.size(1) != 1:
        B, L, D = shape
    else:
        L, B, D = shape[0], 1, shape[2]
    xf = x.float().contiguous()
    tab = None if backward else pe[:L, 0, :].contiguous()
    out = _empty(tuple(shape), _F32, xf)
    _hip.call("mm_add_pe", xf, tab, out, None, B, L, D, float(p), int(seed), EP())
    return out


def transformer_block(x, blk, training, mask=None):
    _need_gpu(x)
    mask = additive_attn_mask(mask, x.shape[1], x)
    if training or (torch.is_grad_enabled() and x.requires_grad):
        from .autograd import TransformerBlockFn
        return TransformerBlockFn.run(blk, x, mask)
    with torch.no_grad():
        return transformer_block_fwd(x.float().contiguous(), blk, False, mask=mask)[0]


def pack_volume(x: torch.Tensor) -> torch.Tensor:
    B, C, D, H, W = x.shape
    if C != 1:
        raise _hip.HipLibraryError("fMRIVolumeEncoder3D: single-channel volumes only")
    y = _empty((B, D, H, W, 16), _BF, x)
    _hip.call("mm_pack_volume_bf16", x.contiguous(), y, B * D * H * W, 16)
    return y


def conv3d_bn_act(xv: torch.Tensor, conv, bn, *, pool: bool, training: bool, drop_p: float,
                  need_dgrad: bool, save=None):
    save = training if save is None else save
    B, D, H, W, cinp = xv.shape
    cout = conv.out_channels
    wf, _, cp, _ = weights.get(conv.weight, need_dgrad)
    assert cp == cinp, (cp, cinp)
    y = _empty((B, D, H, W, cout), _BF if pool else _F32, xv)
    yf, yb = (None, y) if pool else (y, None)
    fin = None
    if training:
        stats = _zeros((REPL, 2, cout), xv)
        cal = kernel_timer.bracket(f"event_pair_c{cinp}")
        if cal is not None:
            cal.record()
        end = kernel_timer.bracket(f"conv3d_fwd_c{cinp}")
        _hip.call("mm_conv3d_fwd", xv, wf, B, D, H, W, cinp, cout, conv.bias, stats, yf, yb)
        if end is not None:
            end.record()
        if cout <= 256:
            fin, out4 = bn_fin_desc(bn, stats, B * D * H * W)
        else:
            out4 = bn_finalize_train(bn, stats, B * D * H * W)
    elif save:
        _hip.call("mm_conv3d_fwd", xv, wf, B, D, H, W, cinp, cout, conv.bias, None, yf, yb)
        out4 = bn_fold_eval(bn, None)
    else:
        _hip.call("mm_conv3d_fwd", xv, wf, B, D, H, W, cinp, cout, None, None, yf, yb)
        out4 = bn_fold_eval(bn, conv.bias)
    seed = _next_seed() if (training and drop_p > 0) else 0
    p = drop_p if training else 0.0
    ysel = arg = None
    fold = training and fin is not None
    if pool:
        out = _empty((B, D // 2, H // 2, W // 2, cout), _BF, xv)
        if save:
            ysel = _empty(out.shape, _BF, xv)
            arg = _empty(out.shape, torch.uint8, xv)
        if fold:
            import ctypes
            _hip.call("mm_pool3d_bn_act_fwd_fin", y, ctypes.addressof(fin), out, ysel, arg, B, D, H, W, cout, ACT["gelu"], float(p), seed, EP())
        else:
            _hip.call("mm_pool3d_bn_act_fwd", y, out4, out, ysel, arg, B, D, H, W, cout, ACT["gelu"], float(p), seed, EP())
    else:
        out = _empty((B, D * H * W, cout), _F32, xv)
        if fold:
            import ctypes
            _hip.call("mm_bn_act_fwd_fin", y, ctypes.addressof(fin), None, None, out, B, D * H * W, cout,
                      ACT["gelu"], 1, 1, float(p), seed, 0.0, 0, EP())
        else:
            _hip.call("mm_bn_act_fwd", y, out4[0], out4[1], None, None, out, B, D * H * W, cout,
                      ACT["gelu"], 1, 1, float(p), seed, 0.0, 0, EP())
    saved = dict(xv=xv, y=y, out4=out4, pool=pool, drop_p=p, seed=seed, conv=conv, bn=bn,
                 ysel=ysel, arg=arg, train=training) if save else None
    return out, saved


def conv3d_l1_bn_act(x: torch.Tensor, conv, bn, *, training: bool, drop_p: float, save=None, winners=None):
    save = training if save is None else save
    B, _, D, H, W = x.shape
    wimg = weights.get(conv.weight.view(32, 27, 1), False, key=conv.weight)[0]
    out = _empty((B, D // 2, H // 2, W // 2, 32), _BF, x)
    p = drop_p if training else 0.0
    seed = _next_seed() if p > 0 else 0
    gramc = fin = None
    if training:
        gram = _zeros((REPL, 32, 32), x)
        stats = _zeros((REPL, 2, 32), x)
        _hip.call("mm_conv3d_l1_gram", x, wimg, conv.bias, gram, stats, B, D, H, W)
        gramc = gram
        if winners is None:
            fin, out4 = bn_fin_desc(bn, stats, B * D * H * W)
        else:
            out4 = bn_finalize_train(bn, stats, B * D * H * W)
        bias = conv.bias
    elif save:
        out4 = bn_fold_eval(bn, None)
        bias = conv.bias
    else:
        out4 = bn_fold_eval(bn, conv.bias)
        bias = None
    if training and fin is not None:
        import ctypes
        _hip.call("mm_conv3d_l1_fwd_fin", x, wimg, bias, ctypes.addressof(fin), out, B, D, H, W, float(p), seed, EP())
    elif winners is not None:
        arg = _empty(tuple(out.shape), torch.uint8, x)
        _hip.call("mm_conv3d_l1_fwd_winners", x, wimg, bias, out4, out, arg, B, D, H, W, 1 if training else 0, float(p), seed, EP())
        winners.append(arg)
    else:
        _hip.call("mm_conv3d_l1", 1, x, wimg, bias, out4, None, None, None, out, None, None,
                  B, D, H, W, 1 if training else 0, float(p), seed, EP())
    saved = dict(l1=True, x=x, wimg=wimg, out4=out4, drop_p=p, seed=seed, conv=conv, bn=bn, train=training, gramc=gramc) if save else None
    return out, saved


def check_volume_shape(shape):
    if len(shape) != 5:
        raise ValueError(f"fMRIVolumeEncoder3D: expected a (B, C, D, H, W) volume batch, got shape {tuple(shape)}")
    if min(shape[2:]) < 4:
        raise ValueError(f"fMRIVolumeEncoder3D: every spatial extent must be >= 4 (two MaxPool3d(2) layers), "
                         f"got D, H, W = {tuple(shape[2:])}")


def _vol_forward_impl(m, x: torch.Tensor, training: bool, need_dgrad: bool, save=None, need_dx: bool = False, winners=None):
    save = training if save is None else save
    cl = m.conv_layers
    p = m.drop_p
    saved = []
    B, C, D, H, W = x.shape
    check_volume_shape(x.shape)
    x = x.contiguous()
    if C == 1 and cl[0].out_channels == 32 and not need_dx:
        h, s = conv3d_l1_bn_act(x, cl[0], cl[1], training=training, drop_p=p, save=save, winners=winners)
    else:
        h, s = conv3d_bn_act(pack_volume(x), cl[0], cl[1], pool=True, training=training, drop_p=p,
                             need_dgrad=need_dgrad or need_dx, save=save)
    saved.append(s)
    h, s = conv3d_bn_act(h, cl[5], cl[6], pool=True, training=training, drop_p=p, need_dgrad=need_dgrad, save=save)
    saved.append(s)
    if winners is not None:
        if len(winners) == 0:
            winners.append(saved[0]["arg"])
        winners.append(s["arg"])
    h, s = conv3d_bn_act(h, cl[10], cl[11], pool=False, training=training, drop_p=p, need_dgrad=need_dgrad, save=save)
    saved.append(s)
    out, hs = pooled_head_fwd(h, m.output_proj[2], training=training, drop_p=p, need_dgrad=need_dgrad, save=save)
    return out, dict(convs=saved, head=hs, x_shape=tuple(x.shape), need_dx=need_dx)


def volume_encoder_forward(m, x: torch.Tensor) -> torch.Tensor:
    check_volume_shape(x.shape)
    _need_gpu(x)
    if m.training or _wants_grad(m, x):
        from .autograd import VolumeEncoderFn
        return VolumeEncoderFn.run(m, x)
    with torch.no_grad():
        return _vol_forward_impl(m, x.float(), False, False)[0]


def small_linear(x: torch.Tensor, lin, *, act="none", drop_p=0.0, seed=0, want_pre=False, bn=None,
                 weight=None, bias=None):
    W = lin.weight if weight is None else weight
    bvec = (lin.bias if lin is not None else None) if bias is None else bias
    B, K = x.shape
    N = W.shape[0]
    y = _empty((B, N), _F32, x)
    pre = _empty((B, N), _F32, x) if want_pre else None
    sc = sh = None
    if bn is not None:
        out4 = bn_fold_eval(bn, None)
        sc, sh = out4[0], out4[1]
    _hip.call("mm_small_linear_fwd", x, W, bvec, sc, sh, y, pre, B, K, N, ACT[act], float(drop_p), int(seed), EP())
    return y, pre

# ... 951 lines not shown
```

Baseline: 41820.

## Store attention dropout keep-bits in forward and reuse them in backward

The forward attention kernel now writes a bitmask of dropout keep decisions to a workspace, computing the hash incrementally. The backward dq and dkv kernels read those bits instead of recomputing the per-element hash. Separately, the grid is flattened and blocks are remapped so that each (batch, head) pair's tiles land on the same XCD. This trades hash ALU work in backward for extra memory traffic of about L*L/8 bytes per head, plus a workspace allocation.

Result: faster. 42360 (median of 6 runs) (+1.3%).

```diff
diff --git a/include/mmeeg_hip.h b/include/mmeeg_hip.h
--- a/include/mmeeg_hip.h
+++ b/include/mmeeg_hip.h
@@ -153,6 +153,15 @@
                    float* delta_ws, int B, int L, int H, int head_dim, float scale, float drop_p,
                    uint32_t seed, const uint32_t* seed_epoch, const float* attn_mask, int attn_mask_per_head,
                    hipStream_t stream);
+
+int mm_attn_fwd_keep(const void* qkv, void* out, float* lse, uint32_t* keep, int B, int L, int H, int head_dim,
+                     float scale, float drop_p, uint32_t seed, const uint32_t* seed_epoch,
+                     const float* attn_mask, int attn_mask_per_head, hipStream_t stream);
+int mm_attn_bwd_keep(const void* qkv, const void* out, const void* dout, const float* lse, void* dqkv,
+                     float* delta_ws, const uint32_t* keep, int B, int L, int H, int head_dim, float scale, float drop_p,
+                     uint32_t seed, const uint32_t* seed_epoch, const float* attn_mask, int attn_mask_per_head,
+                     hipStream_t stream);
+int mm_attn_tile_map(int id, int tiles, int pairs, int* tile_host, int* pair_host, hipStream_t stream);
 
 int mm_colsum(const void* a_bf16, const float* a_f32, float* out, int M, int N, hipStream_t stream);
 int mm_meanpool_fwd(const float* x, float* out_f32, void* out_bf16, int B, int L, int D, hipStream_t stream);
diff --git a/multimodal_eeg_fmri_amd/autograd.py b/multimodal_eeg_fmri_amd/autograd.py
--- a/multimodal_eeg_fmri_amd/autograd.py
+++ b/multimodal_eeg_fmri_amd/autograd.py
@@ -346,8 +346,12 @@
     dh = D // blk.nhead
     pa, sa = s.get("attn_drop", (0.0, 0))
     entry = ops.attn_entry(D, blk.nhead, "bwd")
-    _hip.call(entry, s["qkv"], s["o"], do, s["lse"], dqkv, delta, B, L, blk.nhead, dh, float(dh) ** -0.5,
-              float(pa), int(sa), ops.EP(), s.get("mask"), ops.attn_mask_per_head(s.get("mask"), B, blk.nhead, L))
+    if s.get("keep") is not None:
+        _hip.call("mm_attn_bwd_keep", s["qkv"], s["o"], do, s["lse"], dqkv, delta, s["keep"], B, L, blk.nhead, dh,
+                  float(dh) ** -0.5, float(pa), int(sa), ops.EP(), None, 0)
+    else:
+        _hip.call(entry, s["qkv"], s["o"], do, s["lse"], dqkv, delta, B, L, blk.nhead, dh, float(dh) ** -0.5,
+                  float(pa), int(sa), ops.EP(), s.get("mask"), ops.attn_mask_per_head(s.get("mask"), B, blk.nhead, L))
     dx0 = _empty((M, D), _F32, dx2)
     emit = _empty((M, D), _BF, dx2) if emit_for is not None else None
     ep, es = emit_for if emit_for is not None else (0.0, 0)
diff --git a/multimodal_eeg_fmri_amd/csrc/attention.hip b/multimodal_eeg_fmri_amd/csrc/attention.hip
--- a/multimodal_eeg_fmri_amd/csrc/attention.hip
+++ b/multimodal_eeg_fmri_amd/csrc/attention.hip
@@ -18,13 +18,16 @@
     return (key & ~12) | ((key & 4) << 1) | ((key & 8) >> 1);
 }
 
-__device__ __forceinline__ uint32_t attn_block_hash(uint32_t seed, int bh, int q, int key, int L) {
-    const uint32_t Lh = ((uint32_t)L + 1u) >> 1;
-    uint32_t x = (((uint32_t)bh * Lh + ((uint32_t)q >> 1)) * Lh + ((uint32_t)key >> 1)) * 0x9E3779B1u + seed;
+constexpr uint32_t ATTN_HASH_MUL = 0x9E3779B1u;
+__device__ __forceinline__ uint32_t attn_hash_mix(uint32_t x) {
     x ^= x >> 13;
     x = __umul24(x, 0xB5297Bu);
     x ^= x >> 15;
     return x;
+}
+__device__ __forceinline__ uint32_t attn_block_hash(uint32_t seed, int bh, int q, int key, int L) {
+    const uint32_t Lh = ((uint32_t)L + 1u) >> 1;
+    return attn_hash_mix((((uint32_t)bh * Lh + ((uint32_t)q >> 1)) * Lh + ((uint32_t)key >> 1)) * ATTN_HASH_MUL + seed);
 }
 template <bool ALONG_KEYS>
 __device__ __forceinline__ void attn_keep2(uint32_t seed, int bh, int mine, int other, int L, uint32_t thresh8, bool& k0, bool& k1) {
@@ -39,6 +42,20 @@
     }
 }
 
+__device__ __forceinline__ float keep_and(float v, uint32_t word, uint32_t bit) {
+    return __uint_as_float(__float_as_uint(v) & (uint32_t)__builtin_amdgcn_sbfe((int)word, bit, 1u));
+}
+template <bool FULL>
+__device__ __forceinline__ uint4 keep_load4(const uint32_t* row, int w0, int W) {
+    if (FULL) return *reinterpret_cast<const uint4*>(row + w0);
+    uint4 v = make_uint4(0, 0, 0, 0);
+    if (w0 < W) v.x = row[w0];
+    if (w0 + 1 < W) v.y = row[w0 + 1];
+    if (w0 + 2 < W) v.z = row[w0 + 2];
+    if (w0 + 3 < W) v.w = row[w0 + 3];
+    return v;
+}
+
 __device__ __forceinline__ float xhalf_max(float v) {
     const auto r = __builtin_amdgcn_permlane32_swap(__float_as_uint(v), __float_as_uint(v), false, false);
     return fmaxf(__uint_as_float(r[0]), __uint_as_float(r[1]));
@@ -70,35 +87,41 @@
 
 template <int DHP, bool EXACT>
 struct Dims {
-    int L, H, dh_;
-    Dims(int L, int H, int dh) : L(L), H(H), dh_(dh) {}
+    int L, H, P, dh_;
+    Dims(int L, int H, int P, int dh) : L(L), H(H), P(P), dh_(dh) {}
     __device__ int dh() const { return dh_; }
 };
 template <int DHP>
 struct Dims<DHP, true> {
-    int L, H;
-    Dims(int L, int H, int) : L(L), H(H) {}
+    int L, H, P;
+    Dims(int L, int H, int P, int) : L(L), H(H), P(P) {}
     __device__ constexpr int dh() const { return DHP; }
 };
 
-template <int DHP, bool EXACT, bool DROP, bool FULL, bool MASK>
+template <int DHP, bool EXACT, bool DROP, bool FULL, bool MASK, bool KEEP>
 __global__ __launch_bounds__(256) void attn_fwd_kernel(const bf16* __restrict__ qkv, bf16* __restrict__ out,
                                                        float* __restrict__ lse, const Dims<DHP, EXACT> dm, float scale_log2,
                                                        uint32_t dthresh, uint32_t dseed, float dinv,
-                                                       const uint32_t* epoch, const float* __restrict__ amask, size_t amask_bh) {
+                                                       const uint32_t* epoch, const float* __restrict__ amask, size_t amask_bh,
+                                                       uint32_t* __restrict__ keep) {
+    static_assert(!KEEP || (DROP && !MASK), "keep bits: dropout on, no additive mask");
     using T = Hd<DHP>;
     constexpr int NS = T::NS, NT = T::NT, KS = T::KS, NG = T::NG;
     const int L = dm.L, H = dm.H, dh = dm.dh();
+    const AttnTile tm = attn_tile_map(blockIdx.x, (L + 127) >> 7, dm.P);
     dseed = mm_eff_seed(dseed, epoch);
-    if (MASK) amask += (size_t)(blockIdx.z * H + blockIdx.y) * amask_bh;
+    if (MASK) amask += (size_t)tm.pair * amask_bh;
     __shared__ __attribute__((aligned(16))) bf16 Ks[KCH * KS];
     __shared__ __attribute__((aligned(16))) bf16 Vs[NT * KCH * VR];
     const int E = H * dh, E3 = 3 * E;
-    const int b = blockIdx.z, h = blockIdx.y;
+    const int b = tm.pair / H, h = tm.pair % H;
     const int tid = threadIdx.x, lane = tid & 63, wave = tid >> 6;
     const int lr = lane & 31, lh = lane >> 5;
-    const int q = blockIdx.x * 128 + wave * 32 + lr;
+    const int q = tm.tile * 128 + wave * 32 + lr;
     const bf16* base = qkv + (size_t)b * L * E3 + h * dh;
+    const int W = (L + 31) >> 5;
+    uint4 kacc = make_uint4(0, 0, 0, 0);
+    uint32_t hxt = ((((uint32_t)tm.pair * (((uint32_t)L + 1u) >> 1) + ((uint32_t)q >> 1)) * (((uint32_t)L + 1u) >> 1)) + 2u * lh) * ATTN_HASH_MUL + dseed;
 
     bf16x8 qf[NS];
 #pragma unroll
@@ -188,6 +211,7 @@
             const float m_neg = (MASK && m_run == -INFINITY) ? 0.f : -m_run;
             float ps = 0.f;
             union { bf16x8 v[2]; bf16x2 h[8]; } pu;
+            uint32_t kw = 0;
 #pragma unroll
             for (int r = 0; r < 16; r += 2) {
                 float p0 = fast_exp2(fmaf(sacc[r], sc2, m_neg)), p1 = fast_exp2(fmaf(sacc[r + 1], sc2, m_neg));
@@ -195,17 +219,46 @@
                 ps += p1;
                 if (DROP) {
                     bool kp0, kp1;
-                    attn_keep2<true>(dseed, b * H + h, q, k0 + kt + (r & 3) + 8 * (r >> 2) + 4 * lh, L, dthresh, kp0, kp1);
+                    if (KEEP) {
+                        const uint32_t x = attn_hash_mix(hxt + (uint32_t)(((r & 3) >> 1) + 4 * (r >> 2)) * ATTN_HASH_MUL) >> (16 * (q & 1));
+                        kp0 = (x & 0xFFu) >= dthresh;
+                        kp1 = ((x >> 8) & 0xFFu) >= dthresh;
+                    } else
+                        attn_keep2<true>(dseed, b * H + h, q, k0 + kt + (r & 3) + 8 * (r >> 2) + 4 * lh, L, dthresh, kp0, kp1);
                     p0 = kp0 ? p0 : 0.f; p1 = kp1 ? p1 : 0.f;
+                    if (KEEP) kw |= (kp0 ? 1u << ((r & 3) + 8 * (r >> 2)) : 0u) | (kp1 ? 2u << ((r & 3) + 8 * (r >> 2)) : 0u);
                 }
                 typedef __attribute__((ext_vector_type(2))) float f32x2_t;
                 pu.h[r >> 1] = __builtin_convertvector((f32x2_t){p0, p1}, bf16x2);
             }
             l_run += ps;
+            if (KEEP) {
+                kw <<= 4 * lh;
+                const auto x = __builtin_amdgcn_permlane32_swap(kw, kw, false, false);
+                kw = x[0] | x[1];
+                if (!FULL && kn - kt < 32) kw &= (1u << (kn - kt)) - 1u;
+                kacc = make_uint4(kacc.y, kacc.z, kacc.w, kw);
+                hxt += 16u * ATTN_HASH_MUL;
+            }
 #pragma unroll
             for (int t = 0; t < NT; ++t)
 #pragma unroll
                 for (int s = 0; s < 2; ++s) o[t] = __builtin_amdgcn_mfma_f32_32x32x16_bf16(vfr[t][s], pu.v[s], o[t], 0, 0, 0);
+        }
+        if (KEEP) {
+            if (!FULL)
+                for (int t = kn32; t < KCH; t += 32) kacc = make_uint4(kacc.y, kacc.z, kacc.w, 0u);
+            if (q < L && lh == 0) {
+                uint32_t* kr = keep + ((size_t)tm.pair * L + q) * W;
+                const int w0 = k0 >> 5;
+                if (FULL) *reinterpret_cast<uint4*>(kr + w0) = kacc;
+                else {
+                    if (w0 < W) kr[w0] = kacc.x;
+                    if (w0 + 1 < W) kr[w0 + 1] = kacc.y;
+                    if (w0 + 2 < W) kr[w0 + 2] = kacc.z;
+                    if (w0 + 3 < W) kr[w0 + 3] = kacc.w;
+                }
+            }
         }
     }
     const float l_tot = xhalf_sum(l_run);
@@ -225,27 +278,32 @@
     }
 }
 
-template <int DHP, bool EXACT, bool DROP, bool FULL, bool MASK>
+template <int DHP, bool EXACT, bool DROP, bool FULL, bool MASK, bool KEEP>
 __global__ __launch_bounds__(256) void attn_bwd_dq_kernel(const bf16* __restrict__ qkv, const bf16* __restrict__ out,
                                                           const bf16* __restrict__ dout, const float* __restrict__ lse,
                                                           bf16* __restrict__ dqkv, float* __restrict__ delta,
                                                           const Dims<DHP, EXACT> dm, float scale, uint32_t dthresh,
                                                           uint32_t dseed, float dinv, const uint32_t* epoch,
-                                                          const float* __restrict__ amask, size_t amask_bh) {
+                                                          const float* __restrict__ amask, size_t amask_bh,
+                                                          const uint32_t* __restrict__ keep) {
+    static_assert(!KEEP || (DROP && !MASK), "keep bits: dropout on, no additive mask");
     using T = Hd<DHP>;
     constexpr int NS = T::NS, NT = T::NT, KS = T::KS, NG = T::NG;
     const int L = dm.L, H = dm.H, dh = dm.dh();
+    const AttnTile tm = attn_tile_map(blockIdx.x, (L + 127) >> 7, dm.P);
     dseed = mm_eff_seed(dseed, epoch);
-    if (MASK) amask += (size_t)(blockIdx.z * H + blockIdx.y) * amask_bh;
+    if (MASK) amask += (size_t)tm.pair * amask_bh;
     __shared__ __attribute__((aligned(16))) bf16 Ks[KCH * KS];
     __shared__ __attribute__((aligned(16))) bf16 Vs[KCH * KS];
     __shared__ __attribute__((aligned(16))) bf16 Kr[NT * KCH * VR];
     const int E = H * dh, E3 = 3 * E;
-    const int b = blockIdx.z, h = blockIdx.y;
+    const int b = tm.pair / H, h = tm.pair % H;
     const int tid = threadIdx.x, lane = tid & 63, wave = tid >> 6;
     const int lr = lane & 31, lh = lane >> 5;
-    const int q = blockIdx.x * 128 + wave * 32 + lr;
+    const int q = tm.tile * 128 + wave * 32 + lr;
     const bool qok = q < L;
+    const int W = (L + 31) >> 5;
+    const uint32_t* krow = KEEP ? keep + ((size_t)tm.pair * L + min(q, L - 1)) * W : nullptr;
     const bf16* base = qkv + (size_t)b * L * E3 + h * dh;
     const float scale_log2 = scale * 1.4426950408889634f;
 
@@ -275,6 +333,7 @@
 
     constexpr int NI = KCH * NG / 256;
     uint4 kreg[NI], vreg[NI];
+    uint4 kwreg = make_uint4(0, 0, 0, 0);
     auto load_chunk = [&](int k0) __attribute__((always_inline)) {
         const int kn = min(KCH, L - k0);
 #pragma unroll
@@ -287,6 +346,7 @@
                 vreg[i] = *reinterpret_cast<const uint4*>(row + 2 * E + sg * 8);
             }
         }
+        if (KEEP) kwreg = keep_load4<FULL>(krow, k0 >> 5, W);
     };
     load_chunk(0);
 #pragma unroll
@@ -304,6 +364,7 @@
             *reinterpret_cast<uint4*>(Vs + key * KS + sg * 8) = vreg[i];
             *reinterpret_cast<uint4*>(Kr + T::tr_off(KCH, vperm(key), sg)) = kreg[i];
         }
+        uint4 kwc = make_uint4(kwreg.x >> 4 * lh, kwreg.y >> 4 * lh, kwreg.z >> 4 * lh, kwreg.w >> 4 * lh);
         __syncthreads();
         if (k0 + KCH < L) load_chunk(k0 + KCH);
         for (int kt = 0; kt < kn32; kt += 32) {
@@ -328,7 +389,9 @@
                 for (int s = 0; s < 2; ++s) ktfr[t][s] = tr_frag32(Kr + t * KCH * VR, kt + 16 * s, lane);
             bf16x8 dsf[2];
             bool kp[16];
-            if (DROP)
+            const uint32_t kwt = kwc.x;
+            if (KEEP) kwc = make_uint4(kwc.y, kwc.z, kwc.w, 0u);
+            if (DROP && !KEEP)
 #pragma unroll
                 for (int r = 0; r < 16; r += 2)
                     attn_keep2<true>(dseed, b * H + h, q, k0 + kt + (r & 3) + 8 * (r >> 2) + 4 * lh, L, dthresh, kp[r], kp[r + 1]);
@@ -339,7 +402,8 @@
                 if (MASK && key < kn) sc += amask[(size_t)min(q, L - 1) * L + k0 + key] * 1.4426950408889634f;
                 const float p = (FULL || key < kn) ? fast_exp2(sc) : 0.f;
                 float dpr = dp[r];
-                if (DROP) dpr = fmaf(kp[r] ? dpr : 0.f, dinv, -dl);
+                if (KEEP) dpr = fmaf(keep_and(dpr, kwt, (r & 3) + 8 * (r >> 2)), dinv, -dl);
+                else if (DROP) dpr = fmaf(kp[r] ? dpr : 0.f, dinv, -dl);
                 else dpr -= dl;
                 dsf[r >> 3][r & 7] = (bf16)(p * dpr);
             }
@@ -363,27 +427,32 @@
     }
 }
 
-template <int DHP, bool EXACT, bool DROP, bool FULL, bool MASK>
+template <int DHP, bool EXACT, bool DROP, bool FULL, bool MASK, bool KEEP>
 __global__ __launch_bounds__(256) void attn_bwd_dkv_kernel(const bf16* __restrict__ qkv, const bf16* __restrict__ dout,
                                                            const float* __restrict__ lse, const float* __restrict__ delta,
                                                            bf16* __restrict__ dqkv, const Dims<DHP, EXACT> dm, float scale,
                                                            uint32_t dthresh, uint32_t dseed, float dinv,
-                                                           const uint32_t* epoch, const float* __restrict__ amask, size_t amask_bh) {
+                                                           const uint32_t* epoch, const float* __restrict__ amask, size_t amask_bh,
+                                                           const uint32_t* __restrict__ keep) {
+    static_assert(!KEEP || (DROP && !MASK), "keep bits: dropout on, no additive mask");
     using T = Hd<DHP>;
     constexpr int NS = T::NS, NT = T::NT, KS = T::KS, NG = T::NG;
     const int L = dm.L, H = dm.H, dh = dm.dh();
+    const AttnTile tm = attn_tile_map(blockIdx.x, (L + 127) >> 7, dm.P);
     dseed = mm_eff_seed(dseed, epoch);
-    if (MASK) amask += (size_t)(blockIdx.z * H + blockIdx.y) * amask_bh;
+    if (MASK) amask += (size_t)tm.pair * amask_bh;
     __shared__ __attribute__((aligned(16))) bf16 Qs[QCH * KS];
     __shared__ __attribute__((aligned(16))) bf16 Ds[QCH * KS];
     __shared__ __attribute__((aligned(16))) bf16 Qr[NT * QCH * VR];
     __shared__ __attribute__((aligned(16))) bf16 Dr[NT * QCH * VR];
     __shared__ float Ls[QCH], Dl[QCH];
+    __shared__ __attribute__((aligned(16))) uint32_t Kw[KEEP ? 4 * QCH : 4];
     const int E = H * dh, E3 = 3 * E;
-    const int b = blockIdx.z, h = blockIdx.y;
+    const int b = tm.pair / H, h = tm.pair % H;
     const int tid = threadIdx.x, lane = tid & 63, wave = tid >> 6;
     const int lr = lane & 31, lh = lane >> 5;
-    const int key = blockIdx.x * 128 + wave * 32 + lr;
+    const int key = tm.tile * 128 + wave * 32 + lr;
+    const int W = (L + 31) >> 5;
     const bool kok = key < L;
     const bf16* base = qkv + (size_t)b * L * E3 + h * dh;
     const float scale_log2 = scale * 1.4426950408889634f;
@@ -407,6 +476,7 @@
     static_assert(QCH <= 256, "one lse / delta value per thread");
     uint4 qreg[NI], dreg[NI];
     float lreg = INFINITY, dlreg = 0.f;
+    uint4 kwreg = make_uint4(0, 0, 0, 0);
     auto load_chunk = [&](int q0) __attribute__((always_inline)) {
         const int qn = min(QCH, L - q0);
 #pragma unroll
@@ -421,6 +491,10 @@
         const bool ok = tid < qn;
         lreg = ok ? lse[((size_t)b * H + h) * L + q0 + tid] : INFINITY;
         dlreg = ok ? delta[((size_t)b * H + h) * L + q0 + tid] : 0.f;
+        if (KEEP) {
+            kwreg = make_uint4(0, 0, 0, 0);
+            if (ok) kwreg = keep_load4<FULL>(keep + ((size_t)tm.pair * L + q0 + tid) * W, 4 * tm.tile, W);
+        }
     };
     load_chunk(0);
 #pragma unroll
@@ -439,6 +513,7 @@
             *reinterpret_cast<uint4*>(Dr + T::tr_off(QCH, vperm(qi), sg)) = dreg[i];
         }
         if (tid < qn32) { Ls[tid] = lreg * 1.4426950408889634f; Dl[tid] = dlreg; }
+        if (KEEP && tid < qn32) { Kw[tid] = kwreg.x; Kw[QCH + tid] = kwreg.y; Kw[2 * QCH + tid] = kwreg.z; Kw[3 * QCH + tid] = kwreg.w; }
         __syncthreads();
         if (q0 + QCH < L) load_chunk(q0 + QCH);
         for (int qt = 0; qt < qn32; qt += 32) {
@@ -464,28 +539,48 @@
                     dtar[t][s] = tr_frag32(Dr + t * QCH * VR, qt + 16 * s, lane);
                     qtar[t][s] = tr_frag32(Qr + t * QCH * VR, qt + 16 * s, lane);
                 }
-            bf16x8 pf[2], dsf[2];
+            union { bf16x8 v[2]; bf16x2 h[8]; } pf, dsf;
             bool kp[16];
-            if (DROP)
+            uint32_t kwq[16];
+            if (KEEP)
+#pragma unroll
+                for (int g = 0; g < 4; ++g) {
+                    const uint4 w4 = *reinterpret_cast<const uint4*>(Kw + wave * QCH + qt + 8 * g + 4 * lh);
+                    kwq[4 * g] = w4.x; kwq[4 * g + 1] = w4.y; kwq[4 * g + 2] = w4.z; kwq[4 * g + 3] = w4.w;
+                }
+            if (DROP && !KEEP)
 #pragma unroll
                 for (int r = 0; r < 16; r += 2)
                     attn_keep2<false>(dseed, b * H + h, key, q0 + qt + (r & 3) + 8 * (r >> 2) + 4 * lh, L, dthresh, kp[r], kp[r + 1]);
+            float pk[16], ds[16];
 #pragma unroll
             for (int r = 0; r < 16; ++r) {
                 const int qi = qt + (r & 3) + 8 * (r >> 2) + 4 * lh;
                 float sc = fmaf(sacc[r], scale_log2, -Ls[qi]);
                 if (MASK && kok && qi < qn) sc += amask[(size_t)(q0 + qi) * L + key] * 1.4426950408889634f;
                 const float p = (FULL || kok) ? fast_exp2(sc) : 0.f;
-                pf[r >> 3][r & 7] = (bf16)((!DROP || kp[r]) ? p : 0.f);
-                const float u = DROP ? fmaf(kp[r] ? dp[r] : 0.f, dinv, -Dl[qi]) : dp[r] - Dl[qi];
-                dsf[r >> 3][r & 7] = (bf16)(p * u);
+                float u;
+                if (KEEP) {
+                    pk[r] = keep_and(p, kwq[r], lr);
+                    u = fmaf(keep_and(dp[r], kwq[r], lr), dinv, -Dl[qi]);
+                } else {
+                    pk[r] = (!DROP || kp[r]) ? p : 0.f;
+                    u = DROP ? fmaf(kp[r] ? dp[r] : 0.f, dinv, -Dl[qi]) : dp[r] - Dl[qi];
+                }
+                ds[r] = p * u;
+            }
+            typedef __attribute__((ext_vector_type(2))) float f32x2_t;
+#pragma unroll
+            for (int r = 0; r < 16; r += 2) {
+                pf.h[r >> 1] = __builtin_convertvector((f32x2_t){pk[r], pk[r + 1]}, bf16x2);
+                dsf.h[r >> 1] = __builtin_convertvector((f32x2_t){ds[r], ds[r + 1]}, bf16x2);
             }
 #pragma unroll
             for (int t = 0; t < NT; ++t)
 #pragma unroll
                 for (int s = 0; s < 2; ++s) {
-                    dv[t] = __builtin_amdgcn_mfma_f32_32x32x16_bf16(dtar[t][s], pf[s], dv[t], 0, 0, 0);
-                    dk[t] = __builtin_amdgcn_mfma_f32_32x32x16_bf16(qtar[t][s], dsf[s], dk[t], 0, 0, 0);
+                    dv[t] = __builtin_amdgcn_mfma_f32_32x32x16_bf16(dtar[t][s], pf.v[s], dv[t], 0, 0, 0);
+                    dk[t] = __builtin_amdgcn_mfma_f32_32x32x16_bf16(qtar[t][s], dsf.v[s], dk[t], 0, 0, 0);
                 }
         }
     }
@@ -514,42 +609,49 @@
 
 template <int DHP, bool EXACT>
 void launch_fwd(const void* qkv, void* out, float* lse, int B, int L, int H, int dh, float scale, float drop_p,
-                uint32_t seed, const uint32_t* seed_epoch, const float* attn_mask, int per_head, hipStream_t st) {
+                uint32_t seed, const uint32_t* seed_epoch, const float* attn_mask, int per_head, uint32_t* keep, hipStream_t st) {
     const uint32_t dth = attn_thresh(drop_p);
     const size_t mask_bh = attn_mask && per_head ? (size_t)L * L : 0;
     const bool full = L % KCH == 0;
-    auto kern = dth ? (full ? attn_fwd_kernel<DHP, EXACT, true, true, false> : attn_fwd_kernel<DHP, EXACT, true, false, false>)
-                    : (full ? attn_fwd_kernel<DHP, EXACT, false, true, false> : attn_fwd_kernel<DHP, EXACT, false, false, false>);
-    if (attn_mask) kern = dth ? attn_fwd_kernel<DHP, EXACT, true, false, true> : attn_fwd_kernel<DHP, EXACT, false, false, true>;
-    hipLaunchKernelGGL(kern, dim3(ceil_div(L, 128), H, B), dim3(256), 0, st, (const bf16*)qkv, (bf16*)out, lse,
-                       Dims<DHP, EXACT>(L, H, dh), scale * 1.4426950408889634f, dth, seed, attn_keep_scale(dth), seed_epoch,
-                       attn_mask, mask_bh);
+    auto kern = dth ? (full ? attn_fwd_kernel<DHP, EXACT, true, true, false, false> : attn_fwd_kernel<DHP, EXACT, true, false, false, false>)
+                    : (full ? attn_fwd_kernel<DHP, EXACT, false, true, false, false> : attn_fwd_kernel<DHP, EXACT, false, false, false, false>);
+    if (attn_mask) kern = dth ? attn_fwd_kernel<DHP, EXACT, true, false, true, false> : attn_fwd_kernel<DHP, EXACT, false, false, true, false>;
+    if constexpr (DHP == 32 && EXACT)
+        if (keep) kern = full ? attn_fwd_kernel<32, true, true, true, false, true> : attn_fwd_kernel<32, true, true, false, false, true>;
+    hipLaunchKernelGGL(kern, dim3(ceil_div(L, 128) * H * B), dim3(256), 0, st, (const bf16*)qkv, (bf16*)out, lse,
+                       Dims<DHP, EXACT>(L, H, B * H, dh), scale * 1.4426950408889634f, dth, seed, attn_keep_scale(dth), seed_epoch,
+                       attn_mask, mask_bh, keep);
 }
 
 template <int DHP, bool EXACT>
 int launch_bwd(const void* qkv, const void* out, const void* dout, const float* lse, void* dqkv, float* delta_ws,
                int B, int L, int H, int dh, float scale, float drop_p, uint32_t seed, const uint32_t* seed_epoch,
-               const float* attn_mask, int per_head, hipStream_t st) {
+               const float* attn_mask, int per_head, const uint32_t* keep, hipStream_t st) {
     const uint32_t dth = attn_thresh(drop_p);
     const float dinv = attn_keep_scale(dth);
     const size_t mask_bh = attn_mask && per_head ? (size_t)L * L : 0;
     const bool full = L % KCH == 0 && L % QCH == 0;
-    auto kdq = dth ? (full ? attn_bwd_dq_kernel<DHP, EXACT, true, true, false> : attn_bwd_dq_kernel<DHP, EXACT, true, false, false>)
-                   : (full ? attn_bwd_dq_kernel<DHP, EXACT, false, true, false> : attn_bwd_dq_kernel<DHP, EXACT, false, false, false>);
-    auto kdkv = dth ? (full ? attn_bwd_dkv_kernel<DHP, EXACT, true, true, false> : attn_bwd_dkv_kernel<DHP, EXACT, true, false, false>)
-                    : (full ? attn_bwd_dkv_kernel<DHP, EXACT, false, true, false> : attn_bwd_dkv_kernel<DHP, EXACT, false, false, false>);
+    auto kdq = dth ? (full ? attn_bwd_dq_kernel<DHP, EXACT, true, true, false, false> : attn_bwd_dq_kernel<DHP, EXACT, true, false, false, false>)
+                   : (full ? attn_bwd_dq_kernel<DHP, EXACT, false, true, false, false> : attn_bwd_dq_kernel<DHP, EXACT, false, false, false, false>);
+    auto kdkv = dth ? (full ? attn_bwd_dkv_kernel<DHP, EXACT, true, true, false, false> : attn_bwd_dkv_kernel<DHP, EXACT, true, false, false, false>)
+                    : (full ? attn_bwd_dkv_kernel<DHP, EXACT, false, true, false, false> : attn_bwd_dkv_kernel<DHP, EXACT, false, false, false, false>);
     if (attn_mask) {
-        kdq = dth ? attn_bwd_dq_kernel<DHP, EXACT, true, false, true> : attn_bwd_dq_kernel<DHP, EXACT, false, false, true>;
-        kdkv = dth ? attn_bwd_dkv_kernel<DHP, EXACT, true, false, true> : attn_bwd_dkv_kernel<DHP, EXACT, false, false, true>;
-    }
-    const dim3 grid(ceil_div(L, 128), H, B);
-    const Dims<DHP, EXACT> dm(L, H, dh);
+        kdq = dth ? attn_bwd_dq_kernel<DHP, EXACT, true, false, true, false> : attn_bwd_dq_kernel<DHP, EXACT, false, false, true, false>;
+        kdkv = dth ? attn_bwd_dkv_kernel<DHP, EXACT, true, false, true, false> : attn_bwd_dkv_kernel<DHP, EXACT, false, false, true, false>;
+    }
+    if constexpr (DHP == 32 && EXACT)
+        if (keep) {
+            kdq = full ? attn_bwd_dq_kernel<32, true, true, true, false, true> : attn_bwd_dq_kernel<32, true, true, false, false, true>;
+            kdkv = full ? attn_bwd_dkv_kernel<32, true, true, true, false, true> : attn_bwd_dkv_kernel<32, true, true, false, false, true>;
+        }
+    const dim3 grid(ceil_div(L, 128) * H * B);
+    const Dims<DHP, EXACT> dm(L, H, B * H, dh);
     hipLaunchKernelGGL(kdq, grid, dim3(256), 0, st, (const bf16*)qkv, (const bf16*)out, (const bf16*)dout, lse,
-                       (bf16*)dqkv, delta_ws, dm, scale, dth, seed, dinv, seed_epoch, attn_mask, mask_bh);
+                       (bf16*)dqkv, delta_ws, dm, scale, dth, seed, dinv, seed_epoch, attn_mask, mask_bh, keep);
     int rc = mm_check_launch(EXACT ? "attn_bwd_dq" : "attn_bwd_hd_dq");
     if (rc) return rc;
     hipLaunchKernelGGL(kdkv, grid, dim3(256), 0, st, (const bf16*)qkv, (const bf16*)dout, lse, delta_ws, (bf16*)dqkv,
-                       dm, scale, dth, seed, dinv, seed_epoch, attn_mask, mask_bh);
+                       dm, scale, dth, seed, dinv, seed_epoch, attn_mask, mask_bh, keep);
     return mm_check_launch(EXACT ? "attn_bwd_dkv" : "attn_bwd_hd_dkv");
 }
 
@@ -563,8 +665,40 @@
     MM_REQUIRE(drop_p >= 0.f && drop_p < 1.f, "attn_fwd: drop_p");
     MM_REQUIRE(qkv && out && B > 0 && L > 0 && H > 0, "attn_fwd: null/invalid");
     MM_REQUIRE(head_dim == 32, "attn_fwd: head_dim=%d (kernel is specialised for 32)", head_dim);
-    launch_fwd<32, true>(qkv, out, lse, B, L, H, head_dim, scale, drop_p, seed, seed_epoch, attn_mask, attn_mask_per_head, st);
+    launch_fwd<32, true>(qkv, out, lse, B, L, H, head_dim, scale, drop_p, seed, seed_epoch, attn_mask, attn_mask_per_head, nullptr, st);
     return mm_check_launch("attn_fwd");
+}
+
+#define MM_ATTN_KEEP_REQUIRE(what)                                                                                          \
+    MM_REQUIRE(head_dim == 32, what ": head_dim=%d (the keep-bit kernels are built for 32)", head_dim);                        \
+    MM_REQUIRE(drop_p >= 0.f && drop_p < 1.f && attn_thresh(drop_p) > 0, what ": drop_p=%g (the keep-bit kernels need dropout on)", (double)drop_p); \
+    MM_REQUIRE(!attn_mask, what ": the keep-bit kernels are not built for an additive attn_mask");                             \
+    MM_REQUIRE(keep && (uintptr_t)keep % 16 == 0, what ": keep workspace null or not 16-byte aligned")
+
+int mm_attn_fwd_keep(const void* qkv, void* out, float* lse, uint32_t* keep, int B, int L, int H, int head_dim, float scale,
+                     float drop_p, uint32_t seed, const uint32_t* seed_epoch, const float* attn_mask, int attn_mask_per_head,
+                     hipStream_t st) {
+    MM_REQUIRE(qkv && out && B > 0 && L > 0 && H > 0, "attn_fwd_keep: null/invalid");
+    MM_ATTN_KEEP_REQUIRE("attn_fwd_keep");
+    launch_fwd<32, true>(qkv, out, lse, B, L, H, head_dim, scale, drop_p, seed, seed_epoch, nullptr, attn_mask_per_head, keep, st);
+    return mm_check_launch("attn_fwd_keep");
+}
+
+int mm_attn_bwd_keep(const void* qkv, const void* out, const void* dout, const float* lse, void* dqkv, float* delta_ws,
+                     const uint32_t* keep, int B, int L, int H, int head_dim, float scale, float drop_p, uint32_t seed,
+                     const uint32_t* seed_epoch, const float* attn_mask, int attn_mask_per_head, hipStream_t st) {
+    MM_REQUIRE(qkv && out && dout && lse && dqkv && delta_ws && B > 0 && L > 0 && H > 0, "attn_bwd_keep: null/invalid");
+    MM_ATTN_KEEP_REQUIRE("attn_bwd_keep");
+    return launch_bwd<32, true>(qkv, out, dout, lse, dqkv, delta_ws, B, L, H, head_dim, scale, drop_p, seed, seed_epoch,
+                                nullptr, attn_mask_per_head, keep, st);
+}
+
+int mm_attn_tile_map(int id, int tiles, int pairs, int* tile_host, int* pair_host, hipStream_t) {
+    MM_REQUIRE(tile_host && pair_host && tiles > 0 && pairs > 0 && id >= 0 && id < tiles * pairs, "attn_tile_map: bad args");
+    const AttnTile t = attn_tile_map(id, tiles, pairs);
+    *tile_host = t.tile;
+    *pair_host = t.pair;
+    return 0;
 }
 
 int mm_attn_bwd(const void* qkv, const void* out, const void* dout, const float* lse, void* dqkv, float* delta_ws,
@@ -573,7 +707,7 @@
     MM_REQUIRE(qkv && out && dout && lse && dqkv && delta_ws && B > 0 && L > 0 && H > 0, "attn_bwd: null/invalid");
     MM_REQUIRE(head_dim == 32, "attn_bwd: head_dim=%d (kernel is specialised for 32)", head_dim);
     return launch_bwd<32, true>(qkv, out, dout, lse, dqkv, delta_ws, B, L, H, head_dim, scale, drop_p, seed, seed_epoch,
-                                attn_mask, attn_mask_per_head, st);
+                                attn_mask, attn_mask_per_head, nullptr, st);
 }
 
 int mm_attn_fwd_hd(const void* qkv, void* out, float* lse, int B, int L, int H, int head_dim, float scale,
@@ -583,7 +717,7 @@
     MM_REQUIRE(drop_p >= 0.f && drop_p < 1.f, "attn_fwd_hd: drop_p");
     MM_REQUIRE(qkv && out && B > 0 && L > 0 && H > 0, "attn_fwd_hd: null/invalid");
     auto launch = head_dim <= 32 ? launch_fwd<32, false> : launch_fwd<64, false>;
-    launch(qkv, out, lse, B, L, H, head_dim, scale, drop_p, seed, seed_epoch, attn_mask, attn_mask_per_head, st);
+    launch(qkv, out, lse, B, L, H, head_dim, scale, drop_p, seed, seed_epoch, attn_mask, attn_mask_per_head, nullptr, st);
     return mm_check_launch("attn_fwd_hd");
 }
 
@@ -595,7 +729,7 @@
     MM_REQUIRE(qkv && out && dout && lse && dqkv && delta_ws && B > 0 && L > 0 && H > 0, "attn_bwd_hd: null/invalid");
     auto launch = head_dim <= 32 ? launch_bwd<32, false> : launch_bwd<64, false>;
     return launch(qkv, out, dout, lse, dqkv, delta_ws, B, L, H, head_dim, scale, drop_p, seed, seed_epoch, attn_mask,
-                  attn_mask_per_head, st);
-}
-
-}
+                  attn_mask_per_head, nullptr, st);
+}
+
+}
diff --git a/multimodal_eeg_fmri_amd/csrc/common.h b/multimodal_eeg_fmri_amd/csrc/common.h
--- a/multimodal_eeg_fmri_amd/csrc/common.h
+++ b/multimodal_eeg_fmri_amd/csrc/common.h
@@ -251,6 +251,13 @@
 static inline int ceil_div(int a, int b) { return (a + b - 1) / b; }
 static inline int grid_for(size_t n, int cap) { size_t g = (n + 255) / 256; return (int)(g < (size_t)cap ? (g ? g : 1) : cap); }
 
+struct AttnTile { int tile, pair; };
+__host__ __device__ __forceinline__ AttnTile attn_tile_map(int id, int tiles, int pairs) {
+    if (pairs % 8) return AttnTile{id % tiles, id / tiles};
+    const int xcd = id % 8, slot = id / 8;
+    return AttnTile{slot % tiles, xcd + 8 * (slot / tiles)};
+}
+
 __host__ __device__ __forceinline__ bool conv3d_stream_shape(int rows, int ch) {
     return (rows == 128 && ch == 64) || (rows == 64 && ch == 128) || (rows == 32 && ch == 64);
 }
diff --git a/multimodal_eeg_fmri_amd/ops.py b/multimodal_eeg_fmri_amd/ops.py
--- a/multimodal_eeg_fmri_amd/ops.py
+++ b/multimodal_eeg_fmri_amd/ops.py
@@ -461,7 +461,17 @@
     return round(256.0 * float(p)) / 256.0
 
 
-def attention(qkv: torch.Tensor, nhead: int, want_lse: bool, drop_p: float = 0.0, seed: int = 0, mask=None):
+ATTN_KEEP_BITS = True
+
+
+def attn_keep_workspace(qkv: torch.Tensor, nhead: int, drop_p: float, mask=None):
+    B, L, E3 = qkv.shape
+    if not ATTN_KEEP_BITS or mask is not None or E3 // 3 != 32 * nhead or attn_effective_dropout(drop_p) <= 0.0:
+        return None
+    return _empty((B * nhead, L, (L + 31) // 32), torch.int32, qkv)
+
+
+def attention(qkv: torch.Tensor, nhead: int, want_lse: bool, drop_p: float = 0.0, seed: int = 0, mask=None, keep=None):
     if 0.0 < float(drop_p) < 1.0 / 512.0:
         import warnings
         warnings.warn(f"attention dropout p = {drop_p} is below the kernels' resolution (1/256): no attention-probability dropout "
@@ -472,6 +482,10 @@
     dh = E // nhead
     out = _empty((B, L, E), _BF, qkv)
     lse = _empty((B, nhead, L), _F32, qkv) if want_lse else None
+    if keep is not None:
+        _hip.call("mm_attn_fwd_keep", qkv, out, lse, keep, B, L, nhead, dh, 1.0 / math.sqrt(dh), float(drop_p), int(seed),
+                  EP(), None, 0)
+        return out, lse
     _hip.call(entry, qkv, out, lse, B, L, nhead, dh, 1.0 / math.sqrt(dh), float(drop_p), int(seed), EP(), mask,
               attn_mask_per_head(mask, B, nhead, L))
     return out, lse
@@ -579,7 +593,8 @@
                           need_dgrad=need_dgrad)["bf16"]
     pa = float(blk.self_attn.dropout) if training else 0.0
     sa = _next_seed() if pa > 0 else 0
-    o, lse = attention(qkv.view(B, L, 3 * D), blk.nhead, save, pa, sa, mask)
+    keep = attn_keep_workspace(qkv.view(B, L, 3 * D), blk.nhead, pa, mask) if save else None
+    o, lse = attention(qkv.view(B, L, 3 * D), blk.nhead, save, pa, sa, mask, keep)
     s1 = _next_seed() if p > 0 else 0
     f1 = None
     s2 = None
@@ -645,7 +660,7 @@
     if save:
         saved = dict(x=x2, h1=h1, st1=st1, qkv=qkv, o=o, lse=lse, x1=x1, h2=h2, st2=st2,
                      z=f1["pre"], g=f1["bf16"], p=p, seeds=(s1, s2, s3), attn_drop=(pa, sa), B=B, L=L, blk=blk,
-                     mask=mask)
+                     mask=mask, keep=keep)
     if next_norm is not None:
         return x2o.view(B, L, D), saved, nxt
     return x2o.view(B, L, D), saved
```
